# zsyOAOA/VIRNet

Measured on AMD Instinct MI355X. Metric: images/sec (256x256x3 denoise fwd), higher is better.
Workload: dtype f32 (3x3 conv products as split-fp16 MFMA pairs, f32 accumulate)

## Files before the change

### include/virnet_hip.h

```cpp
#ifndef VIRNET_HIP_H
#define VIRNET_HIP_H

#include <stddef.h>
#include <stdint.h>

#ifdef __cplusplus
extern "C" {
#endif

#define VIRNET_ABI_VERSION 5

int virnet_abi_version(void);
const char* virnet_last_error(void);
int virnet_device_count(void);

size_t virnet_packed_weight_floats(int ks, int cin_pad, int n_pad);
int virnet_pack_weight(const float* w, int kind, int cout, int cin, int ks, int cin_pad, int n_pad, int nrep,
                       float* packed, void* stream);

typedef struct virnet_conv_plan {
  int nrep;
  int n_pad;
  int cin_pad;
} virnet_conv_plan;
int virnet_conv_get_plan(int ks, int stride, int cin, int gemm_n, virnet_conv_plan* plan);

enum { VIRNET_EPI_NHWC = 0, VIRNET_EPI_CONVT = 1, VIRNET_EPI_NCHW = 2 };
enum { VIRNET_NCHW_PLAIN = 0, VIRNET_NCHW_ADD = 1, VIRNET_NCHW_EXPCLAMP = 2 };

typedef struct virnet_conv_desc {
  const float* x;
  const float* wpack;
  const float* bias;
  const float* res;
  const float* mul;
  const float* add;
  const float* mask;
  const float* in_mul;
  const float* in_add;
  float* y_raw;
  float* y_act;
  int n, h, w;
  int cin_pad;
  int cout;
  int n_pad;
  int nrep;
  int ks, stride;
  int epi;
  int nchw_op;
  int crop_h, crop_w;
  int res_sf;
  int in_act;
  float in_slope;
  float slope;
  float mask_slope;
  float clamp_lo, clamp_hi;
} virnet_conv_desc;

int virnet_conv_mfma(const virnet_conv_desc* d, void* stream);
int virnet_conv_mfma_variant(const virnet_conv_desc* d, int out[4]);

size_t virnet_wino_weight_floats(int cin_pad, int n_pad);
int virnet_pack_wino_weight(const float* w_oihw, int dgrad, int cout, int cin, int cin_pad, int n_pad, float* packed, void* stream);
int virnet_conv_wino(const virnet_conv_desc* d, void* stream);

size_t virnet_f16_weight_floats(int cin_pad, int n_pad);
int virnet_pack_f16_weight(const float* w_oihw, int dgrad, int cout, int cin, int cin_pad, int n_pad, float* packed, void* stream);
int virnet_conv_f16(const virnet_conv_desc* d, void* stream);
int virnet_pack_bf16_weight(const float* w_oihw, int dgrad, int cout, int cin, int cin_pad, int n_pad, float* packed, void* stream);
int virnet_conv_bf16(const virnet_conv_desc* d, void* stream);
size_t virnet_f16_convt_weight_floats(int cin, int cout);
int virnet_pack_f16_convt_weight(const float* w_iohw, int cout, int cin, float* packed, void* stream);

size_t virnet_wx4_weight_floats(int cin_pad, int n_pad);
int virnet_pack_wx4_weight(const float* w_oihw, int dgrad, int cout, int cin, int cin_pad, int n_pad, float* packed, void* stream);
int virnet_conv_wx4(const virnet_conv_desc* d, void* stream);
void virnet_conv_wx4_last_plan(int* out4);

enum { VIRNET_LAUNCH_WX4 = 0, VIRNET_LAUNCH_WX4H = 1, VIRNET_LAUNCH_WX4P = 2, VIRNET_LAUNCH_F16 = 3, VIRNET_LAUNCH_S2 = 4, VIRNET_LAUNCH_CONVT = 5 };
typedef struct virnet_conv_launch {
  int form, rows, ng, nrep, variant, slab_base, groups, persistent;
} virnet_conv_launch;
enum { VIRNET_PLAN_WX4 = 0, VIRNET_PLAN_F16 = 1, VIRNET_PLAN_BF16 = 2, VIRNET_PLAN_F16_ENTRY = 3 };
int virnet_conv_plan_query(int family, const virnet_conv_desc* d, int emit_rows, int n_cu,
                           virnet_conv_launch* out, int cap);

size_t virnet_exit_weight_floats(int cin_pad);
int virnet_pack_exit_weight(const float* w_oihw, int cout, int cin, int cin_pad, float* packed, void* stream);
int virnet_conv_exit(const virnet_conv_desc* d, void* stream);

int virnet_set_range_flag(int* device_flag);
int virnet_poison_on_flag(const int* device_flag, float* y, size_t n, void* stream);

typedef struct virnet_thin_desc {
  const float* x;
  const float* wpack;
  const float* bias;
  const float* res;
  float* y;
  int n, h, w, c, cout;
  int crop_h, crop_w;
  int op;
  int res_sf;
  float clamp_lo, clamp_hi;
} virnet_thin_desc;
size_t virnet_thin_weight_floats(int c_pad);
int virnet_pack_thin_weight(const float* w_oihw, int cout, int c, int c_pad, float* packed, void* stream);
int virnet_conv3x3_thin(const virnet_thin_desc* d, void* stream);

typedef struct virnet_pack_desc {
  const float* x;
  const float* vec;
  const float* map;
  float* out;
  int n, c0, h, w, sf;
  int ev;
  int em, mh, mw, msf, map_sqrt;
  int hp, wp;
  int zero_pad;
} virnet_pack_desc;
int virnet_pack_input(const virnet_pack_desc* d, void* stream);
int virnet_conv_f16_entry(const virnet_conv_desc* d, const virnet_pack_desc* e, void* stream);
size_t virnet_entry_weight_floats(int cin, int n_pad);
int virnet_pack_entry_weight(const float* w, int cout, int cin, int n_pad, float* packed, void* stream);
int virnet_conv_entry(const virnet_conv_desc* d, const virnet_pack_desc* e, void* stream);

typedef struct virnet_wgrad_desc {
  const float* x;
  const float* dy;
  const float* in_mul;
  const float* in_add;
  float* dw;
  int* counters;
  int n, h, w, cx, cy;
  int cin, cout;
  int ks, stride;
  int transposed;
  int in_act;
  float in_slope;
} virnet_wgrad_desc;
int virnet_conv_wgrad(const virnet_wgrad_desc* d, void* stream);
size_t virnet_chsplit_bytes(int n, int h, int w, int c);
size_t virnet_conv_wgrad_f16_scratch_bytes(int n, int h, int w, int cx, int cy);
size_t virnet_chsplit_colsum_bytes(int n, int h, int w, int c);
int virnet_chsplit(const float* x, int n, int h, int w, int c, int in_act, float in_slope, const float* in_mul, const float* in_add,
                   int bf16, void* out, float* col_scratch, float* db, int cvalid, void* stream);
int virnet_conv_wgrad_f16(const void* xt, const void* yt, float* dw, float* scratch, int n, int h, int w, int cx, int cy, int cin, int cout,
                          int bf16, void* stream);
int virnet_conv_wgrad_f16_db(const void* xt, const void* yt, float* dw, float* scratch, int n, int h, int w, int cx, int cy, int cin, int cout,
                             int bf16, const float* col, float* db, long nblk, int cvalid, void* stream);
size_t virnet_chsplit_s2_bytes(int n, int h, int w, int c);
size_t virnet_chsplit_s2_colsum_bytes(int n, int h, int w, int c);
int virnet_chsplit_s2(const float* x, int n, int h, int w, int c, int in_act, float in_slope, const float* in_mul, const float* in_add,
                      int bf16, void* out, float* col_scratch, float* db, int cvalid, void* stream);
size_t virnet_conv_wgrad_f16_s2_scratch_bytes(int n, int oh, int ow, int chi, int clo);
int virnet_conv_wgrad_f16_s2(const void* hi_t, const void* lo_t, float* dw, float* scratch, int n, int oh, int ow, int chi, int clo,
                             int cin, int cout, int mode, int bf16, void* stream);
typedef struct {
  int kg, nwv, pairs, split, run, nxs, nsteps;
} virnet_wgrad_f16_plan;
int virnet_conv_wgrad_f16_plan_query(int n, int h, int w, int cx, int cy, int mode, virnet_wgrad_f16_plan* out);
typedef struct virnet_t_emit {
  void* t_out;
  float* col;
  int act;
  float slope;
  int bf16;
  int rows;
} virnet_t_emit;
int virnet_conv_emit_ok(const virnet_conv_desc* d, int form, int* nblk);
int virnet_conv_f16_emit(const virnet_conv_desc* d, const virnet_t_emit* te, int bf16_operands, void* stream);
int virnet_conv_wx4_emit(const virnet_conv_desc* d, const virnet_t_emit* te, void* stream);
int virnet_colpart_reduce(const float* col, float* db, long nblk, int ncb, int cvalid, void* stream);
int virnet_sft_backward(const float* da, const float* x, const float* mul, const float* add, const float* res, float slope, float* dx,
                        float* dmul, float* dadd, int n, long hw, int c, void* stream);
int virnet_colsum(const float* dy, float* db, long npix, int c, int cvalid, void* stream);
int virnet_zero_stuff2(const float* dy, float* z, int n, int h, int w, int c, void* stream);
int virnet_space_to_depth2(const float* dy, float* out, int n, int h, int w, int c, void* stream);
int virnet_pack_input_backward(const float* drec, int crec, int chan, const float* map, float* dmap, int n, int h, int w, int hp,
                               int wp, int map_sqrt, int accumulate, void* stream);

typedef struct virnet_image_grad_desc {
  const float* dres;
  const float* ga;
  const float* wa;
  const float* gb;
  const float* wb;
  float* dx;
  int n, c0, h, w, sf;
  int hp, wp, ca, cina;
  int cb, cinb;
  int accumulate;
} virnet_image_grad_desc;
int virnet_image_grad(const virnet_image_grad_desc* d, void* stream);


int virnet_conv_head_s4(const float* x, const float* w, float* out, int n, int cin, int h, int w_, int cout, void* stream);
int virnet_conv_head_s4_wgrad(const float* x, const float* dy, float* dw, int n, int cin, int h, int w_, int cout, void* stream);
int virnet_conv_head_s4_dgrad(const float* dy, const float* w, float* dx, int n, int cin, int h, int w_, int cout, void* stream);

enum { VIRNET_GAP_MEAN = 0, VIRNET_GAP_EXPCLAMP = 1, VIRNET_GAP_KINFO = 2 };
int virnet_gap_nchw(const float* x, float* out, int n, int c, int h, int w, int finish, float lo, float hi, void* stream);

int virnet_ca_gate(const float* x, const float* w1, const float* b1, const float* w2, const float* b2, float* gate,
                   int n, int h, int w, int c, int cr, void* stream);

int virnet_scale_add(const float* hcv, const float* gate, const float* skip, float* out, int n, int hw, int c, void* stream);

int virnet_ca_scale_add(const float* hcv, const float* w1, const float* b1, const float* w2, const float* b2, const float* skip,
                        float* out, int n, int h, int w, int c, int cr, void* stream);

typedef struct virnet_knet_layer {
  const float *w1pack, *b1, *w2pack, *b2;
  const float *caw1, *cab1, *caw2, *cab2;
} virnet_knet_layer;
int virnet_knet_body(const float* x, float* y, const virnet_knet_layer* layers, int nlayers, int n, int h, int w, int c, int cr, void* stream);

typedef struct virnet_sft_weights {
  const float *w1, *b1;
  const float *w2, *b2;
  const float *wm, *bm;
  const float *wa, *ba;
  int e, nf1, nf2, nf;
} virnet_sft_weights;

int virnet_sft_vec(const float* vec, const virnet_sft_weights* wt, float* mul, float* add, int n, void* stream);
int virnet_sft_vec_multi(const float* vec, const virnet_sft_weights* wts, int nlayers, float* const* muls, float* const* adds, int n, void* stream);

int virnet_sft_apply(const float* raw, const float* rec, const virnet_sft_weights* wt, float* act, int n, int h, int w,
                     int step, int chan0, void* stream);

int virnet_quantize_u8(const float* x, uint8_t* out, size_t n, void* stream);
int virnet_rgb2y_u8(const uint8_t* rgb, uint8_t* y, int n, int h, int w, void* stream);
size_t virnet_psnr_ssim_workspace_bytes(int n, int c, int h, int w, int border, int ycbcr);
int virnet_psnr_ssim(const void* a, int a_f32, const void* b, int b_f32, int n, int c, int h, int w, int border, int ycbcr, int with_ssim,
                     const double* win11, void* workspace, int64_t* sse, int64_t* count, double* ssim, void* stream);

#define VIRNET_BORDER_REFLECT 0
#define VIRNET_BORDER_SYMMETRIC 1
int virnet_degrade_forward(const float* x, const float* kernel, float* y, int n, int c, int h, int w, int k, int sf, int border, int clip01,
                           void* stream);
int virnet_degrade_grad_image(const float* gy, const float* kernel, float* gx, int n, int c, int h, int w, int k, int sf, int border,
                              void* stream);
size_t virnet_degrade_grad_kernel_workspace_bytes(int n, int c, int h, int w, int k, int sf);
int virnet_degrade_grad_kernel(const float* gy, const float* x, float* gk, void* workspace, int n, int c, int h, int w, int k, int sf, int border,
                               void* stream);
int virnet_resample_axis(const void* in, int in_f64, void* out, int out_f64, const int32_t* idx, const double* wgt, int taps, long long outer,
                         int n_in, int n_out, long long inner, void* stream);

size_t virnet_elbo_workspace_bytes(int n, int c, int h, int w);
int virnet_elbo_value(const float* mu, const float* sigma_est, const float* im_noisy, const float* im_gt, const float* beta0,
                      const float* alpha0, const float* psi, float eps2, int with_klig, void* workspace, float* out4, int n, int c, int cs,
                      int cb, int h, int w, void* stream);
int virnet_elbo_grad(const float* mu, const float* sigma_est, const float* im_noisy, const float* im_gt, const float* beta0,
                     const float* alpha0, const float* grad_out, float eps2, double w_data, double w_klig, float* dmu, float* dsigma, int n,
                     int c, int cs, int cb, int h, int w, void* stream);
int virnet_noise_estimate(const float* im_noisy, const float* im_gt, const double* taps, float* out, int n, int c, int h, int w, int k,
                          float floor, void* stream);

size_t virnet_sisr_head_workspace_bytes(int n);
int virnet_sisr_head_forward(const float* kinfo_est, const float* kinfo_gt, const float* gamma, const float* rho_eps, const float* kappa0,
                             double r2, double penalty0, double penalty1, int k, int sf, int shift, void* workspace, float* kernel, float* out4,
                             int n, void* stream);
int virnet_sisr_head_backward(const float* kinfo_est, const float* kinfo_gt, const float* gamma, const float* rho_eps, const float* kappa0,
                              const float* grad_kernel, const float* grad_knet, double r2, double penalty0, double penalty1, int k, int sf,
                              int shift, float* dkinfo, int n, void* stream);
size_t virnet_sisr_hr_workspace_bytes(int n, int c, int h, int w);
int virnet_sisr_hr_value(const float* mu, const float* im_hr, const float* z_eps, double eps2, void* workspace, float* zz, float* out1, int n,
                         int c, int h, int w, void* stream);
int virnet_sisr_hr_grad(const float* mu, const float* im_hr, const float* grad_zz, const float* grad_rnet, double eps2, float* dmu, int n, int c,
                        int h, int w, void* stream);
size_t virnet_sisr_lr_workspace_bytes(int n, int c, int h, int w);
int virnet_sisr_lr_value(const float* y, const float* im_lr, const float* sigma_est, const float* sigma_prior, const float* alpha0,
                         const float* psi, void* workspace, double* stats, float* out2, int n, int c, int h, int w, int cs, int fs, int cp, int fp,
                         void* stream);
int virnet_sisr_lr_grad(const float* y, const float* im_lr, const float* sigma_est, const float* sigma_prior, const float* alpha0,
                        const double* stats, const float* grad_lh, const float* grad_snet, float* dy, float* dsigma, int n, int c, int h, int w,
                        int cs, int fs, int cp, int fp, void* stream);
int virnet_sisr_finish(const float* lh, const float* kl_rnet, const float* kl_snet, const float* kl_knet, float* loss, void* stream);

#ifdef __cplusplus
}
#endif
#endif
```

### virnet_amd/_native.py

```python
from __future__ import annotations

import ctypes as C
import os
import threading

import torch

_HERE = os.path.dirname(os.path.abspath(__file__))
LIB_PATH = os.environ.get("VIRNET_HIP_LIB") or os.path.join(_HERE, "lib", "libvirnet_hip.so")
ABI_VERSION = 5

c_float_p = C.POINTER(C.c_float)


class ConvPlan(C.Structure):
    _fields_ = [("nrep", C.c_int), ("n_pad", C.c_int), ("cin_pad", C.c_int)]


class ConvDesc(C.Structure):
    _fields_ = [
        ("x", C.c_void_p), ("wpack", C.c_void_p), ("bias", C.c_void_p), ("res", C.c_void_p),
        ("mul", C.c_void_p), ("add", C.c_void_p), ("mask", C.c_void_p), ("in_mul", C.c_void_p), ("in_add", C.c_void_p),
        ("y_raw", C.c_void_p), ("y_act", C.c_void_p),
        ("n", C.c_int), ("h", C.c_int), ("w", C.c_int), ("cin_pad", C.c_int), ("cout", C.c_int),
        ("n_pad", C.c_int), ("nrep", C.c_int), ("ks", C.c_int), ("stride", C.c_int), ("epi", C.c_int),
        ("nchw_op", C.c_int), ("crop_h", C.c_int), ("crop_w", C.c_int), ("res_sf", C.c_int),
        ("in_act", C.c_int), ("in_slope", C.c_float), ("slope", C.c_float), ("mask_slope", C.c_float), ("clamp_lo", C.c_float), ("clamp_hi", C.c_float),
    ]


class ConvLaunch(C.Structure):
    _fields_ = [(k, C.c_int) for k in ("form", "rows", "ng", "nrep", "variant", "slab_base", "groups", "persistent")]


class WgradF16Plan(C.Structure):
    _fields_ = [(k, C.c_int) for k in ("kg", "nwv", "pairs", "split", "run", "nxs", "nsteps")]


class TEmit(C.Structure):
    _fields_ = [("t_out", C.c_void_p), ("col", C.c_void_p), ("act", C.c_int), ("slope", C.c_float), ("bf16", C.c_int), ("rows", C.c_int)]


class PackDesc(C.Structure):
    _fields_ = [
        ("x", C.c_void_p), ("vec", C.c_void_p), ("map", C.c_void_p), ("out", C.c_void_p),
        ("n", C.c_int), ("c0", C.c_int), ("h", C.c_int), ("w", C.c_int), ("sf", C.c_int),
        ("ev", C.c_int),
        ("em", C.c_int), ("mh", C.c_int), ("mw", C.c_int), ("msf", C.c_int), ("map_sqrt", C.c_int),
        ("hp", C.c_int), ("wp", C.c_int), ("zero_pad", C.c_int),
    ]


class ImageGradDesc(C.Structure):
    _fields_ = [
        ("dres", C.c_void_p), ("ga", C.c_void_p), ("wa", C.c_void_p), ("gb", C.c_void_p), ("wb", C.c_void_p), ("dx", C.c_void_p),
        ("n", C.c_int), ("c0", C.c_int), ("h", C.c_int), ("w", C.c_int), ("sf", C.c_int),
        ("hp", C.c_int), ("wp", C.c_int), ("ca", C.c_int), ("cina", C.c_int),
        ("cb", C.c_int), ("cinb", C.c_int), ("accumulate", C.c_int),
    ]


class ThinDesc(C.Structure):
    _fields_ = [
        ("x", C.c_void_p), ("wpack", C.c_void_p), ("bias", C.c_void_p), ("res", C.c_void_p), ("y", C.c_void_p),
        ("n", C.c_int), ("h", C.c_int), ("w", C.c_int), ("c", C.c_int), ("cout", C.c_int),
        ("crop_h", C.c_int), ("crop_w", C.c_int), ("op", C.c_int), ("res_sf", C.c_int),
        ("clamp_lo", C.c_float), ("clamp_hi", C.c_float),
    ]


class WgradDesc(C.Structure):
    _fields_ = [
        ("x", C.c_void_p), ("dy", C.c_void_p), ("in_mul", C.c_void_p), ("in_add", C.c_void_p), ("dw", C.c_void_p),
        ("counters", C.c_void_p), ("n", C.c_int), ("h", C.c_int), ("w", C.c_int), ("cx", C.c_int), ("cy", C.c_int),
        ("cin", C.c_int), ("cout", C.c_int), ("ks", C.c_int), ("stride", C.c_int), ("transposed", C.c_int),
        ("in_act", C.c_int), ("in_slope", C.c_float),
    ]


class KnetLayer(C.Structure):
    _fields_ = [(k, C.c_void_p) for k in ("w1pack", "b1", "w2pack", "b2", "caw1", "cab1", "caw2", "cab2")]


class SftWeights(C.Structure):
    _fields_ = [
        ("w1", C.c_void_p), ("b1", C.c_void_p), ("w2", C.c_void_p), ("b2", C.c_void_p),
        ("wm", C.c_void_p), ("bm", C.c_void_p), ("wa", C.c_void_p), ("ba", C.c_void_p),
        ("e", C.c_int), ("nf1", C.c_int), ("nf2", C.c_int), ("nf", C.c_int),
    ]


EPI_NHWC, EPI_CONVT, EPI_NCHW = 0, 1, 2
GAP_MEAN, GAP_EXPCLAMP, GAP_KINFO = 0, 1, 2
NCHW_PLAIN, NCHW_ADD, NCHW_EXPCLAMP = 0, 1, 2
PLAN_WX4, PLAN_F16, PLAN_BF16, PLAN_F16_ENTRY = 0, 1, 2, 3

SYMBOLS = [
    ("virnet_abi_version", C.c_int, []),
    ("virnet_last_error", C.c_char_p, []),
    ("virnet_device_count", C.c_int, []),
    ("virnet_packed_weight_floats", C.c_size_t, [C.c_int, C.c_int, C.c_int]),
    ("virnet_pack_weight", C.c_int, [C.c_void_p, C.c_int, C.c_int, C.c_int, C.c_int, C.c_int, C.c_int, C.c_int,
                                     C.c_void_p, C.c_void_p]),
    ("virnet_conv_get_plan", C.c_int, [C.c_int, C.c_int, C.c_int, C.c_int, C.POINTER(ConvPlan)]),
    ("virnet_conv_mfma", C.c_int, [C.POINTER(ConvDesc), C.c_void_p]),
    ("virnet_conv_mfma_variant", C.c_int, [C.POINTER(ConvDesc), C.POINTER(C.c_int * 4)]),
    ("virnet_wino_weight_floats", C.c_size_t, [C.c_int, C.c_int]),
    ("virnet_pack_wino_weight", C.c_int, [C.c_void_p, C.c_int, C.c_int, C.c_int, C.c_int, C.c_int, C.c_void_p, C.c_void_p]),
    ("virnet_conv_wino", C.c_int, [C.POINTER(ConvDesc), C.c_void_p]),
    ("virnet_f16_weight_floats", C.c_size_t, [C.c_int, C.c_int]),
    ("virnet_pack_f16_weight", C.c_int, [C.c_void_p, C.c_int, C.c_int, C.c_int, C.c_int, C.c_int, C.c_void_p, C.c_void_p]),
    ("virnet_conv_f16", C.c_int, [C.POINTER(ConvDesc), C.c_void_p]),
    ("virnet_wx4_weight_floats", C.c_size_t, [C.c_int, C.c_int]),
    ("virnet_pack_wx4_weight", C.c_int, [C.c_void_p, C.c_int, C.c_int, C.c_int, C.c_int, C.c_int, C.c_void_p, C.c_void_p]),
    ("virnet_conv_wx4", C.c_int, [C.POINTER(ConvDesc), C.c_void_p]),
    ("virnet_conv_wx4_last_plan", None, [C.POINTER(C.c_int)]),
    ("virnet_conv_plan_query", C.c_int, [C.c_int, C.POINTER(ConvDesc), C.c_int, C.c_int, C.POINTER(ConvLaunch), C.c_int]),
    ("virnet_exit_weight_floats", C.c_size_t, [C.c_int]),
    ("virnet_pack_exit_weight", C.c_int, [C.c_void_p, C.c_int, C.c_int, C.c_int, C.c_void_p, C.c_void_p]),
    ("virnet_conv_exit", C.c_int, [C.POINTER(ConvDesc), C.c_void_p]),
    ("virnet_set_range_flag", C.c_int, [C.c_void_p]),
    ("virnet_poison_on_flag", C.c_int, [C.c_void_p, C.c_void_p, C.c_size_t, C.c_void_p]),
    ("virnet_pack_bf16_weight", C.c_int, [C.c_void_p, C.c_int, C.c_int, C.c_int, C.c_int, C.c_int, C.c_void_p, C.c_void_p]),
    ("virnet_conv_bf16", C.c_int, [C.POINTER(ConvDesc), C.c_void_p]),
    ("virnet_f16_convt_weight_floats", C.c_size_t, [C.c_int, C.c_int]),
    ("virnet_pack_f16_convt_weight", C.c_int, [C.c_void_p, C.c_int, C.c_int, C.c_void_p, C.c_void_p]),
    ("virnet_pack_input", C.c_int, [C.POINTER(PackDesc), C.c_void_p]),
    ("virnet_conv_f16_entry", C.c_int, [C.POINTER(ConvDesc), C.POINTER(PackDesc), C.c_void_p]),
    ("virnet_entry_weight_floats", C.c_size_t, [C.c_int, C.c_int]),
    ("virnet_pack_entry_weight", C.c_int, [C.c_void_p, C.c_int, C.c_int, C.c_int, C.c_void_p, C.c_void_p]),
    ("virnet_conv_entry", C.c_int, [C.POINTER(ConvDesc), C.POINTER(PackDesc), C.c_void_p]),
    ("virnet_thin_weight_floats", C.c_size_t, [C.c_int]),
    ("virnet_pack_thin_weight", C.c_int, [C.c_void_p, C.c_int, C.c_int, C.c_int, C.c_void_p, C.c_void_p]),
    ("virnet_conv3x3_thin", C.c_int, [C.POINTER(ThinDesc), C.c_void_p]),
    ("virnet_conv_wgrad", C.c_int, [C.POINTER(WgradDesc), C.c_void_p]),
    ("virnet_sft_backward", C.c_int, [C.c_void_p, C.c_void_p, C.c_void_p, C.c_void_p, C.c_void_p, C.c_float, C.c_void_p, C.c_void_p, C.c_void_p,
                                      C.c_int, C.c_long, C.c_int, C.c_void_p]),
    ("virnet_chsplit_bytes", C.c_size_t, [C.c_int, C.c_int, C.c_int, C.c_int]),
    ("virnet_conv_wgrad_f16_scratch_bytes", C.c_size_t, [C.c_int, C.c_int, C.c_int, C.c_int, C.c_int]),
    ("virnet_chsplit_colsum_bytes", C.c_size_t, [C.c_int, C.c_int, C.c_int, C.c_int]),
    ("virnet_chsplit", C.c_int, [C.c_void_p, C.c_int, C.c_int, C.c_int, C.c_int, C.c_int, C.c_float, C.c_void_p, C.c_void_p, C.c_int,
                                 C.c_void_p, C.c_void_p, C.c_void_p, C.c_int, C.c_void_p]),
    ("virnet_conv_wgrad_f16", C.c_int, [C.c_void_p, C.c_void_p, C.c_void_p, C.c_void_p, C.c_int, C.c_int, C.c_int, C.c_int, C.c_int, C.c_int, C.c_int,
                                        C.c_int, C.c_void_p]),
    ("virnet_chsplit_s2_bytes", C.c_size_t, [C.c_int, C.c_int, C.c_int, C.c_int]),
    ("virnet_chsplit_s2_colsum_bytes", C.c_size_t, [C.c_int, C.c_int, C.c_int, C.c_int]),
    ("virnet_chsplit_s2", C.c_int, [C.c_void_p, C.c_int, C.c_int, C.c_int, C.c_int, C.c_int, C.c_float, C.c_void_p, C.c_void_p, C.c_int,
                                    C.c_void_p, C.c_void_p, C.c_void_p, C.c_int, C.c_void_p]),
    ("virnet_conv_wgrad_f16_s2_scratch_bytes", C.c_size_t, [C.c_int, C.c_int, C.c_int, C.c_int, C.c_int]),
    ("virnet_conv_wgrad_f16_s2", C.c_int, [C.c_void_p, C.c_void_p, C.c_void_p, C.c_void_p, C.c_int, C.c_int, C.c_int, C.c_int, C.c_int, C.c_int,
                                           C.c_int, C.c_int, C.c_int, C.c_void_p]),
    ("virnet_conv_wgrad_f16_plan_query", C.c_int, [C.c_int, C.c_int, C.c_int, C.c_int, C.c_int, C.c_int, C.POINTER(WgradF16Plan)]),
    ("virnet_conv_emit_ok", C.c_int, [C.POINTER(ConvDesc), C.c_int, C.POINTER(C.c_int)]),
    ("virnet_conv_f16_emit", C.c_int, [C.POINTER(ConvDesc), C.POINTER(TEmit), C.c_int, C.c_void_p]),
    ("virnet_conv_wx4_emit", C.c_int, [C.POINTER(ConvDesc), C.POINTER(TEmit), C.c_void_p]),
    ("virnet_colpart_reduce", C.c_int, [C.c_void_p, C.c_void_p, C.c_long, C.c_int, C.c_int, C.c_void_p]),
    ("virnet_conv_wgrad_f16_db", C.c_int, [C.c_void_p, C.c_void_p, C.c_void_p, C.c_void_p, C.c_int, C.c_int, C.c_int, C.c_int, C.c_int, C.c_int, C.c_int,
                                           C.c_int, C.c_void_p, C.c_void_p, C.c_long, C.c_int, C.c_void_p]),
    ("virnet_colsum", C.c_int, [C.c_void_p, C.c_void_p, C.c_long, C.c_int, C.c_int, C.c_void_p]),
    ("virnet_zero_stuff2", C.c_int, [C.c_void_p, C.c_void_p, C.c_int, C.c_int, C.c_int, C.c_int, C.c_void_p]),
    ("virnet_space_to_depth2", C.c_int, [C.c_void_p, C.c_void_p, C.c_int, C.c_int, C.c_int, C.c_int, C.c_void_p]),
    ("virnet_pack_input_backward", C.c_int, [C.c_void_p, C.c_int, C.c_int, C.c_void_p, C.c_void_p, C.c_int, C.c_int, C.c_int, C.c_int,
                                             C.c_int, C.c_int, C.c_int, C.c_void_p]),
    ("virnet_image_grad", C.c_int, [C.POINTER(ImageGradDesc), C.c_void_p]),
    ("virnet_conv_head_s4", C.c_int, [C.c_void_p, C.c_void_p, C.c_void_p, C.c_int, C.c_int, C.c_int, C.c_int, C.c_int,
                                      C.c_void_p]),
    ("virnet_conv_head_s4_wgrad", C.c_int, [C.c_void_p, C.c_void_p, C.c_void_p, C.c_int, C.c_int, C.c_int, C.c_int, C.c_int,
                                            C.c_void_p]),
    ("virnet_conv_head_s4_dgrad", C.c_int, [C.c_void_p, C.c_void_p, C.c_void_p, C.c_int, C.c_int, C.c_int, C.c_int, C.c_int,
                                            C.c_void_p]),
    ("virnet_gap_nchw", C.c_int, [C.c_void_p, C.c_void_p, C.c_int, C.c_int, C.c_int, C.c_int, C.c_int, C.c_float,
                                  C.c_float, C.c_void_p]),
    ("virnet_ca_gate", C.c_int, [C.c_void_p, C.c_void_p, C.c_void_p, C.c_void_p, C.c_void_p, C.c_void_p, C.c_int, C.c_int,
                                 C.c_int, C.c_int, C.c_int, C.c_void_p]),
    ("virnet_knet_body", C.c_int, [C.c_void_p, C.c_void_p, C.c_void_p, C.c_int, C.c_int, C.c_int, C.c_int, C.c_int, C.c_int, C.c_void_p]),
    ("virnet_scale_add", C.c_int, [C.c_void_p, C.c_void_p, C.c_void_p, C.c_void_p, C.c_int, C.c_int, C.c_int, C.c_void_p]),
    ("virnet_ca_scale_add", C.c_int, [C.c_void_p] * 7 + [C.c_int] * 5 + [C.c_void_p]),
    ("virnet_sft_vec", C.c_int, [C.c_void_p, C.POINTER(SftWeights), C.c_void_p, C.c_void_p, C.c_int, C.c_void_p]),
    ("virnet_sft_vec_multi", C.c_int, [C.c_void_p, C.POINTER(SftWeights), C.c_int, C.POINTER(C.c_void_p), C.POINTER(C.c_void_p), C.c_int, C.c_void_p]),
    ("virnet_sft_apply", C.c_int, [C.c_void_p, C.c_void_p, C.POINTER(SftWeights), C.c_void_p, C.c_int, C.c_int, C.c_int,
                                   C.c_int, C.c_int, C.c_void_p]),
    ("virnet_quantize_u8", C.c_int, [C.c_void_p, C.c_void_p, C.c_size_t, C.c_void_p]),
    ("virnet_rgb2y_u8", C.c_int, [C.c_void_p, C.c_void_p, C.c_int, C.c_int, C.c_int, C.c_void_p]),
    ("virnet_psnr_ssim_workspace_bytes", C.c_size_t, [C.c_int] * 6),
    ("virnet_psnr_ssim", C.c_int, [C.c_void_p, C.c_int, C.c_void_p, C.c_int] + [C.c_int] * 7 + [C.POINTER(C.c_double)] + [C.c_void_p] * 5),
    ("virnet_degrade_forward", C.c_int, [C.c_void_p] * 3 + [C.c_int] * 8 + [C.c_void_p]),
    ("virnet_degrade_grad_image", C.c_int, [C.c_void_p] * 3 + [C.c_int] * 7 + [C.c_void_p]),
    ("virnet_degrade_grad_kernel_workspace_bytes", C.c_size_t, [C.c_int] * 6),
    ("virnet_degrade_grad_kernel", C.c_int, [C.c_void_p] * 4 + [C.c_int] * 7 + [C.c_void_p]),
    ("virnet_resample_axis", C.c_int, [C.c_void_p, C.c_int, C.c_void_p, C.c_int, C.c_void_p, C.c_void_p, C.c_int, C.c_longlong, C.c_int, C.c_int,
                                       C.c_longlong, C.c_void_p]),
    ("virnet_elbo_workspace_bytes", C.c_size_t, [C.c_int] * 4),
    ("virnet_elbo_value", C.c_int, [C.c_void_p] * 7 + [C.c_float, C.c_int, C.c_void_p, C.c_void_p] + [C.c_int] * 6 + [C.c_void_p]),
    ("virnet_elbo_grad", C.c_int, [C.c_void_p] * 7 + [C.c_float, C.c_double, C.c_double, C.c_void_p, C.c_void_p] + [C.c_int] * 6 + [C.c_void_p]),
    ("virnet_noise_estimate", C.c_int, [C.c_void_p] * 4 + [C.c_int] * 5 + [C.c_float, C.c_void_p]),
    ("virnet_sisr_head_workspace_bytes", C.c_size_t, [C.c_int]),
    ("virnet_sisr_head_forward", C.c_int, [C.c_void_p] * 5 + [C.c_double] * 3 + [C.c_int] * 3 + [C.c_void_p] * 3 + [C.c_int, C.c_void_p]),
    ("virnet_sisr_head_backward", C.c_int, [C.c_void_p] * 7 + [C.c_double] * 3 + [C.c_int] * 3 + [C.c_void_p, C.c_int, C.c_void_p]),
    ("virnet_sisr_hr_workspace_bytes", C.c_size_t, [C.c_int] * 4),
    ("virnet_sisr_hr_value", C.c_int, [C.c_void_p] * 3 + [C.c_double] + [C.c_void_p] * 3 + [C.c_int] * 4 + [C.c_void_p]),
    ("virnet_sisr_hr_grad", C.c_int, [C.c_void_p] * 4 + [C.c_double, C.c_void_p] + [C.c_int] * 4 + [C.c_void_p]),
    ("virnet_sisr_lr_workspace_bytes", C.c_size_t, [C.c_int] * 4),
    ("virnet_sisr_lr_value", C.c_int, [C.c_void_p] * 9 + [C.c_int] * 8 + [C.c_void_p]),
    ("virnet_sisr_lr_grad", C.c_int, [C.c_void_p] * 10 + [C.c_int] * 8 + [C.c_void_p]),
    ("virnet_sisr_finish", C.c_int, [C.c_void_p] * 6),
]

_lib = None


class NativeLibraryError(RuntimeError):
    pass


def load() -> C.CDLL:
    global _lib
    if _lib is not None:
        return _lib
    if not os.path.exists(LIB_PATH):
        raise NativeLibraryError(
            f"{LIB_PATH} not found: the VIRNet HIP kernels are not built. Run `python -c 'import __graft_entry__ as g; "
            f"g.build()'` (or `make -C virnet_amd/csrc`) -- there is no CPU fallback for the product path.")
    lib = C.CDLL(LIB_PATH)
    for name, restype, argtypes in SYMBOLS:
        try:
            fn = getattr(lib, name)
        except AttributeError as e:
            raise NativeLibraryError(f"{LIB_PATH} does not export {name}; rebuild it") from e
        fn.restype = restype
        fn.argtypes = argtypes
    if lib.virnet_abi_version() != ABI_VERSION:
        raise NativeLibraryError(f"{LIB_PATH}: ABI {lib.virnet_abi_version()} != expected {ABI_VERSION}; rebuild it")
    _lib = lib
    return lib


def check(rc: int, what: str = "") -> None:
    if rc != 0:
        msg = load().virnet_last_error()
        raise RuntimeError(f"libvirnet_hip {what}: {msg.decode() if msg else 'unknown error'}")


def ptr(t) -> int:
    return 0 if t is None else t.data_ptr()


tls = threading.local()
capture_lock = threading.RLock()


def stream_handle() -> int:
    cached = getattr(tls, "stream_cache", None)
    if cached is not None:
        return cached
    return torch.cuda.current_stream().cuda_stream
```

### virnet_amd/csrc/conv_exit.hip

```cpp
#include "conv_f16_common.h"

namespace {
using namespace virnet;

constexpr int EX_TH = 8, EX_TW = 32;
constexpr int EX_HW = EX_TW + 2;
constexpr int EX_HPX = (EX_TH + 2) * EX_HW;
constexpr int EX_BLK = (EX_HPX + 31) / 32;
constexpr int EX_ZS = EX_BLK * 32 + 4;

template <int NCH>
__global__ __launch_bounds__(256) void conv_exit_kernel(const FArgs a) {
  extern __shared__ __attribute__((aligned(16))) char smem[];
  const int nch = NCH ? NCH : (a.Cin >> 4);
  char* const a_lds = smem;
  float* const z_lds = reinterpret_cast<float*>(smem + nch * 2048);

  const int xcd = blockIdx.x & 7, q = blockIdx.x >> 3;
  const int tile = xcd * a.tiles_per_xcd + q;
  if (q >= a.tiles_per_xcd || tile >= a.ntiles) return;
  const int img = fast_div(tile, a.mg_tpi);
  const int trem = tile - img * (a.ntx * a.nty);
  const int ty = fast_div(trem, a.mg_ntx), tx = trem - ty * a.ntx;
  const int oy0 = ty * EX_TH, ox0 = tx * EX_TW;

  const int tid = threadIdx.x, lane = tid & 63, wave = __builtin_amdgcn_readfirstlane(tid >> 6);
  const int l31 = lane & 31, lhi = lane >> 5;
  const int nrows = a.cout * 9;
  TSTAMP(0);

  if constexpr (NCH != 0) {
    f32x4 wv[NCH / 2];
#pragma unroll
    for (int i = 0; i < NCH / 2; ++i) wv[i] = *reinterpret_cast<const f32x4*>(a.wimg + i * 4096 + tid * 16);
#pragma unroll
    for (int i = 0; i < NCH / 2; ++i) *reinterpret_cast<f32x4*>(a_lds + i * 4096 + tid * 16) = wv[i];
  } else {
    for (int i = tid * 16; i < nch * 2048; i += 256 * 16) *reinterpret_cast<f32x4*>(a_lds + i) = *reinterpret_cast<const f32x4*>(a.wimg + i);
  }
  __syncthreads();
  TSTAMP(1);

  const int oyl = tid >> 5, oxl = tid & 31;
  const int oy = oy0 + oyl, ox = ox0 + oxl;
  const bool inside = oy < a.crop_h && ox < a.crop_w;
  const size_t plane = (size_t)a.crop_h * a.crop_w;
  const size_t o0 = (size_t)img * a.cout * plane + (size_t)oy * a.crop_w + ox;
  float scv[27], bsv[3];
#pragma unroll
  for (int i = 0; i < 27; ++i) scv[i] = a.inv_scale[i];
#pragma unroll
  for (int c = 0; c < 3; ++c) bsv[c] = (a.bias && c < a.cout) ? a.bias[c] : 0.f;
  float rv[3] = {0.f, 0.f, 0.f};
  if (a.nchw_op == VIRNET_NCHW_ADD && inside) {
    const int rw = a.crop_w / a.res_sf;
    const size_t rplane = (size_t)(a.crop_h / a.res_sf) * rw;
    const size_t r0 = (size_t)img * a.cout * rplane + (size_t)(oy / a.res_sf) * rw + ox / a.res_sf;
#pragma unroll
    for (int c = 0; c < 3; ++c)
      if (c < a.cout) rv[c] = a.res[a.res_sf > 1 ? r0 + c * rplane : o0 + c * plane];
  }

  const float* const ximg = a.x + (size_t)img * a.H * a.W * a.Cin;
  float amax = 0.f;
  auto pixel_of = [&](int blk) -> const float* {
    const int p = blk * 32 + l31;
    const int hy = p / EX_HW, hx = p - hy * EX_HW;
    const int gy = oy0 - 1 + hy, gx = ox0 - 1 + hx;
    const bool valid = blk < EX_BLK && p < EX_HPX && (unsigned)gy < (unsigned)a.H && (unsigned)gx < (unsigned)a.W;
    return valid ? ximg + ((size_t)gy * a.W + gx) * a.Cin + lhi * 8 : nullptr;
  };
  auto mma = [&](f32x16& acc, int c, f32x4 v0, f32x4 v1) {
    if (a.in_act) { v0 = lrelu4(v0, a.in_slope); v1 = lrelu4(v1, a.in_slope); }
    range_note(amax, v0, v1);
    h8 bh, bl;
    split8(v0, v1, bh, bl);
    const h8 ah = *reinterpret_cast<const h8*>(a_lds + c * 2048 + lane * 16);
    const h8 al = *reinterpret_cast<const h8*>(a_lds + c * 2048 + 1024 + lane * 16);
    acc = __builtin_amdgcn_mfma_f32_32x32x16_f16(al, bh, acc, 0, 0, 0);
    acc = __builtin_amdgcn_mfma_f32_32x32x16_f16(ah, bl, acc, 0, 0, 0);
    acc = __builtin_amdgcn_mfma_f32_32x32x16_f16(ah, bh, acc, 0, 0, 0);
  };
  auto put_z = [&](int blk, const f32x16& acc) {
    const int p = blk * 32 + l31;
#pragma unroll
    for (int r = 0; r < 16; ++r) {
      const int row = 8 * (r >> 2) + 4 * lhi + (r & 3);
      z_lds[min(row, nrows) * EX_ZS + p] = acc[r];
    }
  };
  if constexpr (NCH != 0) {
    const auto xrs = __builtin_amdgcn_make_buffer_rsrc(const_cast<float*>(ximg), 0, a.H * a.W * a.Cin * 4, 0x00020000);
    auto pixel_off = [&](int blk) -> unsigned {
      const int p = blk * 32 + l31;
      const int hy = p / EX_HW, hx = p - hy * EX_HW;
      const int gy = oy0 - 1 + hy, gx = ox0 - 1 + hx;
      const bool valid = p < EX_HPX && (unsigned)gy < (unsigned)a.H && (unsigned)gx < (unsigned)a.W;
      return valid ? (unsigned)(((gy * a.W + gx) * a.Cin + lhi * 8) * 4) : 0x80000000u;
    };
    auto request = [&](unsigned off, f32x4 (&v0)[NCH], f32x4 (&v1)[NCH]) {
#pragma unroll
      for (int c = 0; c < NCH; ++c) {
        v0[c] = __builtin_bit_cast(f32x4, __builtin_amdgcn_raw_buffer_load_b128(xrs, off + c * 64, 0, 0));
        v1[c] = __builtin_bit_cast(f32x4, __builtin_amdgcn_raw_buffer_load_b128(xrs, off + c * 64 + 16, 0, 0));
      }
    };
    auto compute = [&](int blk, f32x4 (&v0)[NCH], f32x4 (&v1)[NCH]) {
      f32x16 acc;
#pragma unroll
      for (int r = 0; r < 16; ++r) acc[r] = 0.f;
#pragma unroll
      for (int c = 0; c < NCH; ++c) mma(acc, c, v0[c], v1[c]);
      put_z(blk, acc);
    };
    static_assert(EX_BLK > 8 && EX_BLK <= 12, "three blocks per wave at most, two at least");
    f32x4 p0[NCH], p1[NCH], q0[NCH], q1[NCH];
    const bool third = wave + 8 < EX_BLK;
    request(pixel_off(wave), p0, p1);
    request(pixel_off(wave + 4), q0, q1);
    compute(wave, p0, p1);
    if (third) request(pixel_off(wave + 8), p0, p1);
    compute(wave + 4, q0, q1);
    if (third) compute(wave + 8, p0, p1);
  } else {
    for (int blk = wave; blk < EX_BLK; blk += 4) {
      const float* const px = pixel_of(blk);
      f32x16 acc;
#pragma unroll
      for (int r = 0; r < 16; ++r) acc[r] = 0.f;
      for (int c = 0; c < nch; ++c) {
        f32x4 v0 = f32x4{0.f, 0.f, 0.f, 0.f}, v1 = v0;
        if (px) {
          v0 = *reinterpret_cast<const f32x4*>(px + c * 16);
          v1 = *reinterpret_cast<const f32x4*>(px + c * 16 + 4);
        }
        mma(acc, c, v0, v1);
      }
      put_z(blk, acc);
    }
  }
  TSTAMP(2);
  range_report(a.range_flag, amax);
  __syncthreads();
  TSTAMP(3);
#ifdef VIRNET_F16_TIMING
  if (a.tlog && tid == 0) {
    a.tlog[(size_t)blockIdx.x * 8 + 5] = __builtin_amdgcn_s_getreg((31 << 11) | (0 << 6) | 4);
    a.tlog[(size_t)blockIdx.x * 8 + 6] = __builtin_amdgcn_s_getreg((31 << 11) | (0 << 6) | 20);
  }
#endif

  if (!inside) return;
  float outv[3];
#pragma unroll
  for (int c = 0; c < 3; ++c) {
    float v = bsv[c];
    const float* const zc = z_lds + (c < a.cout ? c * 9 : 0) * EX_ZS + oyl * EX_HW + oxl;
#pragma unroll
    for (int dy = 0; dy < 3; ++dy)
#pragma unroll
      for (int dx = 0; dx < 3; ++dx) v += zc[(dy * 3 + dx) * EX_ZS + dy * EX_HW + dx] * scv[c * 9 + dy * 3 + dx];
    if (a.nchw_op == VIRNET_NCHW_ADD) v += rv[c];
    else if (a.nchw_op == VIRNET_NCHW_EXPCLAMP) v = expf(fminf(fmaxf(v, a.clamp_lo), a.clamp_hi));
    outv[c] = v;
  }
#pragma unroll
  for (int c = 0; c < 3; ++c)
    if (c < a.cout) a.y_raw[o0 + c * plane] = outv[c];
#ifdef VIRNET_F16_TIMING
  asm volatile("s_waitcnt vmcnt(0)" ::: "memory");
#endif
  TSTAMP(4);
}

__global__ void pack_exit_kernel(const float* __restrict__ w, int cout, int cin, int cin_pad, float* __restrict__ inv_scale, char* __restrict__ img) {
  const int nrows = cout * 9;
  __shared__ int eb[32];
  if (threadIdx.x < 32) {
    const int row = threadIdx.x;
    float m = 0.f;
    if (row < nrows) {
      const int c = row / 9, t = row - c * 9;
      for (int k = 0; k < cin; ++k) m = fmaxf(m, fabsf(w[((size_t)c * cin + k) * 9 + t]));
    }
    int e = 0;
    if (m > 0.f) { frexpf(m, &e); e = 14 - e; }
    e = max(-100, min(100, e));
    eb[row] = e;
    inv_scale[row] = ldexpf(1.f, -e);
  }
  __syncthreads();
  for (int i = threadIdx.x; i < 32 * cin_pad; i += blockDim.x) {
    const int row = i / cin_pad, k = i - row * cin_pad;
    float v = 0.f;
    if (row < nrows && k < cin) {
      const int c = row / 9, t = row - c * 9;
      v = ldexpf(w[((size_t)c * cin + k) * 9 + t], eb[row]);
    }
    const int chunk = k >> 4, kk = k & 15;
    const size_t base = (size_t)chunk * 2048 + (size_t)(row + 32 * (kk >> 3)) * 16 + (kk & 7) * 2;
    const _Float16 hi = (_Float16)v;
    *reinterpret_cast<_Float16*>(img + base) = hi;
    *reinterpret_cast<_Float16*>(img + base + 1024) = (_Float16)(v - (float)hi);
  }
}

template <int NCH>
int launch_exit(FArgs k, hipStream_t st) {
  const int nch = k.Cin >> 4;
  const int lds = nch * 2048 + (k.cout * 9 + 1) * EX_ZS * 4;
  static unsigned long long attr_done = 0;
  auto kern = conv_exit_kernel<NCH>;
  if (virnet::first_use_on_device(attr_done)) {
    hipError_t e = hipFuncSetAttribute(reinterpret_cast<const void*>(kern), hipFuncAttributeMaxDynamicSharedMemorySize, 160 * 1024);
    if (e != hipSuccess) return virnet::set_error("hipFuncSetAttribute(conv_exit): %s", hipGetErrorString(e));
  }
  hipLaunchKernelGGL(kern, dim3((unsigned)(8 * k.tiles_per_xcd)), dim3(256), lds, st, k);
  return virnet::check_launch("conv_exit launch");
}

#ifdef VIRNET_F16_TIMING
long long* g_xlog = nullptr;
#endif
}

#ifdef VIRNET_F16_TIMING
extern "C" void virnet_debug_exit_timing_buffer(void* p) { g_xlog = static_cast<long long*>(p); }
#endif

extern "C" size_t virnet_exit_weight_floats(int cin_pad) { return 32 + (size_t)cin_pad * 32; }

extern "C" int virnet_pack_exit_weight(const float* w, int cout, int cin, int cin_pad, float* packed, void* stream) {
  VIRNET_REQUIRE(w && packed, "virnet_pack_exit_weight: NULL pointer");
  VIRNET_REQUIRE(cout >= 1 && cout * 9 <= 32, "virnet_pack_exit_weight: cout=%d: the (channel, tap) rows must fit one 32-row block (cout <= 3)", cout);
  VIRNET_REQUIRE(cin >= 1 && cin_pad % 16 == 0 && cin_pad >= cin, "virnet_pack_exit_weight: cin_pad=%d does not cover cin=%d", cin_pad, cin);
  hipLaunchKernelGGL(pack_exit_kernel, dim3(1), dim3(256), 0, static_cast<hipStream_t>(stream), w, cout, cin, cin_pad, packed,
                     reinterpret_cast<char*>(packed + 32));
  return virnet::check_launch("pack_exit launch");
}

extern "C" int virnet_conv_exit(const virnet_conv_desc* d, void* stream) {
  VIRNET_REQUIRE(d != nullptr, "virnet_conv_exit: desc is NULL");
  VIRNET_REQUIRE(d->x && d->wpack && d->y_raw, "virnet_conv_exit: x / wpack / y_raw is NULL");
  VIRNET_REQUIRE(d->ks == 3 && d->stride == 1 && d->epi == VIRNET_EPI_NCHW, "virnet_conv_exit: only the stride-1 3x3 conv with planar store (ks=%d stride=%d epi=%d)",
                 d->ks, d->stride, d->epi);
  VIRNET_REQUIRE(d->n > 0 && d->h > 0 && d->w > 0, "virnet_conv_exit: empty input n=%d h=%d w=%d", d->n, d->h, d->w);
  VIRNET_REQUIRE(d->cout >= 1 && d->cout * 9 <= 32, "virnet_conv_exit: cout=%d (the (channel, tap) rows must fit one 32-row block: cout <= 3)", d->cout);
  VIRNET_REQUIRE(d->cin_pad >= 16 && d->cin_pad % 16 == 0 && d->cin_pad <= 1024, "virnet_conv_exit: cin_pad=%d", d->cin_pad);
  VIRNET_REQUIRE(d->crop_h >= 1 && d->crop_h <= d->h && d->crop_w >= 1 && d->crop_w <= d->w, "virnet_conv_exit: crop %d x %d outside %d x %d", d->crop_h, d->crop_w, d->h, d->w);
  VIRNET_REQUIRE(d->nchw_op != VIRNET_NCHW_ADD || d->res, "virnet_conv_exit: VIRNET_NCHW_ADD without res");
  VIRNET_REQUIRE(d->res_sf >= 1 && d->crop_h % d->res_sf == 0 && d->crop_w % d->res_sf == 0, "virnet_conv_exit: res_sf=%d does not divide the crop", d->res_sf);
  VIRNET_REQUIRE(!d->mask && !d->mul && !d->in_mul && !d->y_act, "virnet_conv_exit: plain planar epilogue only");
  VIRNET_REQUIRE((long)d->h * d->w * d->cin_pad * 4 < (1L << 31), "virnet_conv_exit: one image's input (%d x %d x %d fp32) must stay below 2 GB (32-bit buffer offsets)", d->h, d->w, d->cin_pad);
  FArgs k{};
  k.x = d->x; k.inv_scale = d->wpack; k.wimg = reinterpret_cast<const char*>(d->wpack + 32);
  k.bias = d->bias; k.res = d->res; k.y_raw = d->y_raw;
  k.N = d->n; k.H = d->h; k.W = d->w; k.Cin = d->cin_pad; k.cout = d->cout;
  k.in_act = d->in_act; k.in_slope = d->in_slope;
  k.nchw_op = d->nchw_op; k.crop_h = d->crop_h; k.crop_w = d->crop_w; k.res_sf = d->res_sf; k.clamp_lo = d->clamp_lo; k.clamp_hi = d->clamp_hi;
  k.range_flag = virnet::range_flag_ptr();
#ifdef VIRNET_F16_TIMING
  k.tlog = g_xlog;
#endif
  k.nty = (d->crop_h + EX_TH - 1) / EX_TH;
  k.ntx = (d->crop_w + EX_TW - 1) / EX_TW;
  k.ntiles = k.N * k.nty * k.ntx;
  k.tiles_per_xcd = (k.ntiles + 7) / 8;
  VIRNET_REQUIRE((unsigned long long)k.ntiles * (unsigned)(k.ntx * k.nty) < (1ull << 32), "virnet_conv_exit: %d tiles exceed the index arithmetic of one launch", k.ntiles);
  k.mg_ntx = div_magic(k.ntx);
  k.mg_tpi = div_magic(k.ntx * k.nty);
  hipStream_t st = static_cast<hipStream_t>(stream);
  const int nch = d->cin_pad >> 4;
  if (nch == 6) return launch_exit<6>(k, st);
  if (nch == 4) return launch_exit<4>(k, st);
  VIRNET_REQUIRE(nch * 2048 + 33 * EX_ZS * 4 <= 160 * 1024, "virnet_conv_exit: cin_pad=%d does not fit LDS", d->cin_pad);
  return launch_exit<0>(k, st);
}
```

### virnet_amd/csrc/pack.hip

```cpp
#include "common.h"
#include "../../include/virnet_hip.h"

namespace {

__global__ void pack_weight_kernel(const float* __restrict__ w, float* __restrict__ out, int kind, int cout, int cin, int ks,
                                   int cin_pad, int n_pad, int nrep, size_t total) {
  const int ntaps = ks * ks;
  const int nchunks = cin_pad / 16;
  for (size_t i = (size_t)blockIdx.x * blockDim.x + threadIdx.x; i < total; i += (size_t)gridDim.x * blockDim.x) {
    size_t r = i;
    const int rr = (int)(r & 3); r >>= 2;
    const int lane = (int)(r & 63); r >>= 6;
    const int nr = (int)(r % nrep); r /= nrep;
    const int j = (int)(r & 1); r >>= 1;
    const int t = (int)(r % ntaps); r /= ntaps;
    const int c = (int)(r % nchunks); r /= nchunks;
    const int cb = (int)r;
    const int ci = c * 16 + 8 * j + 4 * (lane >> 5) + rr;
    const int n = (cb * nrep + nr) * 32 + (lane & 31);
    float v = 0.f;
    if (kind == 0) {
      if (ci < cin && n < cout) v = w[((size_t)n * cin + ci) * ntaps + t];
    } else if (kind == 1) {
      const int ab = n / cout, co = n - ab * cout;
      if (ci < cin && ab < 4) v = w[((size_t)ci * cout + co) * 4 + ab];
    } else if (kind == 2) {
      if (ci < cout && n < cin) v = w[((size_t)ci * cin + n) * ntaps + (ntaps - 1 - t)];
    } else {
      const int ab = ci / cout, co = ci - ab * cout;
      if (n < cin && ab < 4) v = w[((size_t)n * cout + co) * 4 + ab];
    }
    out[i] = v;
  }
}

__device__ __forceinline__ int reflect(int i, int n) { return i < n ? i : 2 * n - 2 - i; }

__global__ void pack_input_kernel(const virnet_pack_desc d) {
  const size_t npix = (size_t)d.n * d.hp * d.wp;
  const int HU = d.h * d.sf, WU = d.w * d.sf;
  for (size_t i = (size_t)blockIdx.x * blockDim.x + threadIdx.x; i < npix * 4; i += (size_t)gridDim.x * blockDim.x) {
    const int q = (int)(i & 3);
    const size_t pix = i >> 2;
    const int x = (int)(pix % d.wp);
    const int y = (int)((pix / d.wp) % d.hp);
    const int n = (int)(pix / ((size_t)d.wp * d.hp));
    const int ry = reflect(y, HU), rx = reflect(x, WU);
    const bool dead = d.zero_pad && (y >= HU || x >= WU);
    float v[4];
#pragma unroll
    for (int k = 0; k < 4; ++k) {
      int c = q * 4 + k;
      float val = 0.f;
      if (c < d.c0) {
        val = d.x[(((size_t)n * d.c0 + c) * d.h + ry / d.sf) * d.w + rx / d.sf];
      } else if ((c -= d.c0) < d.ev) {
        val = d.vec[(size_t)n * d.ev + c];
      } else if ((c -= d.ev) < d.em) {
        val = d.map[(((size_t)n * d.em + c) * d.mh + ry / d.msf) * d.mw + rx / d.msf];
        if (d.map_sqrt) val = sqrtf(val);
      }
      v[k] = dead ? 0.f : val;
    }
    reinterpret_cast<float4*>(d.out)[i] = make_float4(v[0], v[1], v[2], v[3]);
  }
}

__global__ void zero_stuff2_kernel(const float4* __restrict__ dy, float4* __restrict__ z, int h, int w, int c4, size_t total) {
  for (size_t i = (size_t)blockIdx.x * blockDim.x + threadIdx.x; i < total; i += (size_t)gridDim.x * blockDim.x) {
    const int q = (int)(i % c4);
    size_t p = i / c4;
    const int x = (int)(p % (2 * w)); p /= 2 * w;
    const int y = (int)(p % (2 * h));
    const size_t n = p / (2 * h);
    float4 v = make_float4(0.f, 0.f, 0.f, 0.f);
    if (!((x | y) & 1)) v = dy[((n * h + (y >> 1)) * w + (x >> 1)) * c4 + q];
    z[i] = v;
  }
}

__global__ void space_to_depth2_kernel(const float4* __restrict__ dy, float4* __restrict__ out, int h, int w, int c4, size_t total) {
  for (size_t i = (size_t)blockIdx.x * blockDim.x + threadIdx.x; i < total; i += (size_t)gridDim.x * blockDim.x) {
    const int q = (int)(i % c4);
    size_t p = i / c4;
    const int ab = (int)(p & 3); p >>= 2;
    const int x = (int)(p % w); p /= w;
    const int y = (int)(p % h);
    const size_t n = p / h;
    out[i] = dy[((n * 2 * h + 2 * y + (ab >> 1)) * 2 * w + 2 * x + (ab & 1)) * c4 + q];
  }
}

__global__ void pack_input_backward_kernel(const float* __restrict__ drec, int crec, int chan, const float* __restrict__ map,
                                           float* __restrict__ dmap, int h, int w, int hp, int wp, int map_sqrt, int accumulate,
                                           size_t total) {
  for (size_t i = (size_t)blockIdx.x * blockDim.x + threadIdx.x; i < total; i += (size_t)gridDim.x * blockDim.x) {
    const int x = (int)(i % w), y = (int)((i / w) % h);
    const size_t n = i / ((size_t)w * h);
    const int ym = 2 * h - 2 - y, xm = 2 * w - 2 - x;
    const bool my = ym >= h && ym < hp, mx = xm >= w && xm < wp;
    const float* base = drec + (n * hp * (size_t)wp) * crec + chan;
    float g = base[((size_t)y * wp + x) * crec];
    if (my) g += base[((size_t)ym * wp + x) * crec];
    if (mx) g += base[((size_t)y * wp + xm) * crec];
    if (my && mx) g += base[((size_t)ym * wp + xm) * crec];
    if (map_sqrt) g *= 0.5f / sqrtf(map[i]);
    dmap[i] = accumulate ? dmap[i] + g : g;
  }
}

}

static int grid_for(size_t total) { return (int)((total + 255) / 256 > 8192 ? 8192 : (total + 255) / 256); }

extern "C" int virnet_zero_stuff2(const float* dy, float* z, int n, int h, int w, int c, void* stream) {
  VIRNET_REQUIRE(dy && z && n > 0 && h > 0 && w > 0 && c > 0 && c % 4 == 0, "virnet_zero_stuff2: bad arguments");
  const size_t total = (size_t)n * 2 * h * 2 * w * (c / 4);
  hipLaunchKernelGGL(zero_stuff2_kernel, dim3(grid_for(total)), dim3(256), 0, static_cast<hipStream_t>(stream),
                     reinterpret_cast<const float4*>(dy), reinterpret_cast<float4*>(z), h, w, c / 4, total);
  return virnet::check_launch("zero_stuff2 launch");
}

extern "C" int virnet_space_to_depth2(const float* dy, float* out, int n, int h, int w, int c, void* stream) {
  VIRNET_REQUIRE(dy && out && n > 0 && h > 0 && w > 0 && c > 0 && c % 4 == 0, "virnet_space_to_depth2: bad arguments");
  const size_t total = (size_t)n * h * w * 4 * (c / 4);
  hipLaunchKernelGGL(space_to_depth2_kernel, dim3(grid_for(total)), dim3(256), 0, static_cast<hipStream_t>(stream),
                     reinterpret_cast<const float4*>(dy), reinterpret_cast<float4*>(out), h, w, c / 4, total);
  return virnet::check_launch("space_to_depth2 launch");
}

extern "C" int virnet_pack_input_backward(const float* drec, int crec, int chan, const float* map, float* dmap, int n, int h, int w,
                                          int hp, int wp, int map_sqrt, int accumulate, void* stream) {
  VIRNET_REQUIRE(drec && dmap && n > 0 && h > 0 && w > 0 && hp >= h && wp >= w && hp - h < h && wp - w < w,
                 "virnet_pack_input_backward: bad shape %dx%d -> %dx%d", h, w, hp, wp);
  VIRNET_REQUIRE(chan >= 0 && chan < crec, "virnet_pack_input_backward: channel %d of %d", chan, crec);
  VIRNET_REQUIRE(!map_sqrt || map, "virnet_pack_input_backward: map_sqrt without map");
  const size_t total = (size_t)n * h * w;
  hipLaunchKernelGGL(pack_input_backward_kernel, dim3(grid_for(total)), dim3(256), 0, static_cast<hipStream_t>(stream), drec, crec,
                     chan, map, dmap, h, w, hp, wp, map_sqrt, accumulate, total);
  return virnet::check_launch("pack_input_backward launch");
}

extern "C" size_t virnet_packed_weight_floats(int ks, int cin_pad, int n_pad) {
  return (size_t)ks * ks * cin_pad * n_pad;
}

extern "C" int virnet_pack_weight(const float* w, int kind, int cout, int cin, int ks, int cin_pad, int n_pad, int nrep,
                                  float* packed, void* stream) {
  VIRNET_REQUIRE(w && packed, "virnet_pack_weight: NULL pointer");
  VIRNET_REQUIRE(kind >= 0 && kind <= 3, "virnet_pack_weight: kind=%d", kind);
  VIRNET_REQUIRE(nrep >= 1 && n_pad % (32 * nrep) == 0 && cin_pad % 16 == 0, "virnet_pack_weight: n_pad=%d nrep=%d cin_pad=%d", n_pad, nrep, cin_pad);
  const int rows = kind == 0 ? cout : kind == 1 ? 4 * cout : cin;
  const int contr = kind <= 1 ? cin : kind == 2 ? cout : 4 * cout;
  VIRNET_REQUIRE(n_pad >= rows && cin_pad >= contr, "virnet_pack_weight: n_pad=%d / cin_pad=%d do not cover %d rows x %d channels (kind %d)",
                 n_pad, cin_pad, rows, contr, kind);
  VIRNET_REQUIRE((kind == 1 || kind == 3) ? ks == 2 : (ks == 3 || ks == 1), "virnet_pack_weight: ks=%d for kind %d", ks, kind);
  const int gemm_ks = (kind == 1 || kind == 3) ? 1 : ks;
  const size_t total = virnet_packed_weight_floats(gemm_ks, cin_pad, n_pad);
  const int grid = (int)((total + 255) / 256 > 4096 ? 4096 : (total + 255) / 256);
  hipLaunchKernelGGL(pack_weight_kernel, dim3(grid), dim3(256), 0, static_cast<hipStream_t>(stream), w, packed, kind, cout, cin,
                     gemm_ks, cin_pad, n_pad, nrep, total);
  return virnet::check_launch("pack_weight launch");
}

extern "C" int virnet_pack_input(const virnet_pack_desc* d, void* stream) {
  VIRNET_REQUIRE(d && d->x && d->out, "virnet_pack_input: NULL pointer");
  VIRNET_REQUIRE(d->n > 0 && d->h > 0 && d->w > 0 && d->sf >= 1, "virnet_pack_input: bad shape n=%d h=%d w=%d sf=%d", d->n, d->h,
                 d->w, d->sf);
  VIRNET_REQUIRE(d->c0 >= 1 && d->ev >= 0 && d->em >= 0 && d->c0 + d->ev + d->em <= 16,
                 "virnet_pack_input: %d+%d+%d channels do not fit a 16-channel record", d->c0, d->ev, d->em);
  VIRNET_REQUIRE(d->ev == 0 || d->vec, "virnet_pack_input: ev=%d without vec", d->ev);
  VIRNET_REQUIRE(d->em == 0 || (d->map && d->msf >= 1), "virnet_pack_input: em=%d without map/msf", d->em);
  const int HU = d->h * d->sf, WU = d->w * d->sf;
  VIRNET_REQUIRE(d->hp >= HU && d->wp >= WU && d->hp - HU < HU && d->wp - WU < WU,
                 "virnet_pack_input: reflect pad %dx%d -> %dx%d needs pad < dim", HU, WU, d->hp, d->wp);
  VIRNET_REQUIRE(d->em == 0 || (d->mh * d->msf == HU && d->mw * d->msf == WU),
                 "virnet_pack_input: map %dx%d x%d does not match image %dx%d", d->mh, d->mw, d->msf, HU, WU);
  const size_t total = (size_t)d->n * d->hp * d->wp * 4;
  const int grid = (int)((total + 255) / 256 > 8192 ? 8192 : (total + 255) / 256);
  hipLaunchKernelGGL(pack_input_kernel, dim3(grid), dim3(256), 0, static_cast<hipStream_t>(stream), *d);
  return virnet::check_launch("pack_input launch");
}
```

### virnet_amd/engine.py

```python
from __future__ import annotations

from typing import List, Optional, Tuple

import torch

from . import _native as nat
from . import ops

Tensor = torch.Tensor

LOG_MAX = 4.605170185988092
LOG_MIN = -23.025850929940457
K_LOG_MIN = -9.210340371976182


def _prep(x: Tensor, chn: int, name: str = "x") -> Tensor:
    if x.dim() != 4:
        raise ValueError(f"{name} must be [N,C,H,W], got {tuple(x.shape)}")
    if x.shape[1] != chn:
        raise ValueError(f"{name} has {x.shape[1]} channels, the network was built for {chn}")
    if not x.is_cuda:
        raise RuntimeError(f"{name} is on {x.device}: the VIRNet HIP path runs on a ROCm device only (no CPU fallback)")
    if x.dtype != torch.float32:
        raise TypeError(f"{name} must be float32 (the reference is fp32 end to end), got {x.dtype}")
    return x.detach().contiguous()


def _ceil_to(v: int, m: int) -> int:
    return (v + m - 1) // m * m


def snet_forward(snet, x: Tensor, mode: str = "raw") -> Tensor:
    x = _prep(x, snet.in_channels)
    n, _, h, w = x.shape
    cur = ops.conv_entry(x, snet.conv1.packed(), h, w, want_act=True, slope=0.25)
    for key in sorted(snet.mid_layer.keys(), key=int):
        _, cur = ops.conv_mfma(cur, snet.mid_layer[key].packed(), want_raw=False, want_act=True, slope=0.25)
    last = snet.conv_last
    if snet.noise_avg:
        raw = ops.conv_planar(cur, last, (h, w))
        fin = ops.GAP_EXPCLAMP if mode == "sigma" else ops.GAP_MEAN
        return ops.gap_nchw(raw, fin, (LOG_MIN, LOG_MAX)).view(n, -1, 1, 1)
    if mode == "sigma":
        return ops.conv_planar(cur, last, (h, w), op=nat.NCHW_EXPCLAMP, clamp=(LOG_MIN, LOG_MAX))
    return ops.conv_planar(cur, last, (h, w))


def knet_forward(knet, x: Tensor) -> Tensor:
    x = _prep(x, knet.in_nc)
    n, _, h, w = x.shape
    cur = ops.conv_head_s4(x, knet.head.weight)
    persistent = (ops._f16_family() and cur.shape[3] == 64 and max(cur.shape[1:3]) <= ops.KNET_BODY_MAX and len(knet.body) > 0
                  and ops._env("VIRNET_KNET_PERSISTENT", "1") != "0")
    if persistent:
        cur = ops.knet_body(cur, [(rb.body["0"].packed(), rb.body["2"].packed(), rb.body["3"].body["0"].weight, rb.body["3"].body["0"].bias,
                                   rb.body["3"].body["2"].weight, rb.body["3"].body["2"].bias) for rb in knet.body])
    for rb in (() if persistent else knet.body):
        _, a = ops.conv_mfma(cur, rb.body["0"].packed(), want_raw=False, want_act=True, slope=0.2)
        hcv, _ = ops.conv_mfma(a, rb.body["2"].packed(), want_raw=True)
        ca = rb.body["3"].body
        cur = ops.ca_scale_add(hcv, ca["0"].weight, ca["0"].bias, ca["2"].weight, ca["2"].bias, cur)
    oh, ow = cur.shape[1:3]
    raw = ops.conv_planar(cur, knet.tail["0"], (oh, ow))
    return ops.gap_nchw(raw, ops.GAP_KINFO, (K_LOG_MIN, LOG_MAX)).view(n, -1, 1, 1)


class _Cond:

    def __init__(self, vec: Optional[Tensor], rec: Optional[Tensor], chan0: int, nchan: int):
        self.vec, self.rec, self.chan0, self.nchan = vec, rec, chan0, nchan
        self.pre = {}

    def sft(self, att):
        got = self.pre.get(id(att))
        return got if got is not None else ops.sft_vec(self.vec, att)


def _res_block(x_raw: Tensor, blk, cond: Optional[_Cond], level: int) -> Tensor:
    sft = cond is not None and blk.extra_chn > 0
    c1, c2 = blk.conv1.packed(), blk.conv2.packed()
    if not sft:
        _, f1a = ops.conv_mfma(x_raw, c1, in_slope=0.2, want_raw=False, want_act=True, slope=0.2)
    elif cond.vec is not None:
        mul1, add1 = cond.sft(blk.sft1)
        mul2, add2 = cond.sft(blk.sft2)
        _, f1a = ops.conv_mfma(x_raw, c1, in_slope=0.2, in_mul=mul1, in_add=add1, mul=mul2, add=add2, want_raw=False,
                               want_act=True, slope=0.2)
    else:
        a1 = ops.sft_apply(x_raw, cond.rec, cond.chan0, cond.nchan, 1 << level, blk.sft1)
        f1, _ = ops.conv_mfma(a1, c1, want_raw=True)
        f1a = ops.sft_apply(f1, cond.rec, cond.chan0, cond.nchan, 1 << level, blk.sft2)
    out, _ = ops.conv_mfma(f1a, c2, res=x_raw, want_raw=True)
    return out


def rnet_forward(rnet, x_in: Tensor, *, extra_map: Optional[Tensor] = None, extra_vec: Optional[Tensor] = None,
                 sf: int = 1, map_sf: int = 1, map_sqrt: bool = False) -> Tensor:
    x_in = _prep(x_in, rnet.in_chn)
    mode = rnet.extra_mode
    n, _, h0, w0 = x_in.shape
    H, W = h0 * sf, w0 * sf
    m = 1 << (rnet.depth - 1)
    Hp, Wp = _ceil_to(H, m), _ceil_to(W, m)
    ev = 0 if extra_vec is None else extra_vec.shape[1]
    em = 0 if extra_map is None else extra_map.shape[1]
    if mode != "null":
        if ev + em != rnet.extra_chn:
            raise ValueError(f"conditioning has {ev + em} channels, the network was built for {rnet.extra_chn}")
        if extra_map is not None:
            extra_map = _prep(extra_map, em, "extra maps")
        if extra_vec is not None:
            extra_vec = extra_vec.detach().contiguous()
    feed_head = mode in ("input", "both")
    feed_down = mode in ("down", "both")
    cond = None
    rec = None
    if feed_down:
        if extra_map is None:
            cond = _Cond(extra_vec, None, 0, ev)
        else:
            rec = ops.pack_input(x_in, Hp, Wp, sf=sf, vec=extra_vec if feed_head else None,
                                 map_=extra_map if feed_head else None, map_sf=map_sf, map_sqrt=map_sqrt)
            crec = rec if feed_head else ops.pack_input(x_in, Hp, Wp, sf=sf, vec=extra_vec, map_=extra_map,
                                                        map_sf=map_sf, map_sqrt=map_sqrt)
            cond = _Cond(None, crec, rnet.in_chn, ev + em)
    if rec is not None:
        x, _ = ops.conv_mfma(rec, rnet.head.packed(), want_raw=True)
    else:
        x = ops.conv_entry(x_in, rnet.head.packed(), Hp, Wp, sf=sf, vec=extra_vec if feed_head else None,
                           map_=extra_map if feed_head else None, map_sf=map_sf, map_sqrt=map_sqrt)
    if cond is not None and cond.vec is not None and ops._env("VIRNET_SFT_MULTI", "1") != "0":
        atts = [a for lvl in rnet.down_path for blk in lvl.body if blk.extra_chn > 0 for a in (blk.sft1, blk.sft2)]
        if atts:
            cond.pre = {id(a): ma for a, ma in zip(atts, ops.sft_vec_multi(cond.vec, atts))}
    bridges: List[Tensor] = []
    for ii, lvl in enumerate(rnet.down_path):
        for blk in lvl.body:
            x = _res_block(x, blk, cond, ii)
        if ii + 1 < len(rnet.down_path):
            bridges.append(x)
            x, _ = ops.conv_mfma(x, lvl.downsampler.packed(), stride=2, want_raw=True)
    for jj, up in enumerate(rnet.up_path):
        x, _ = ops.conv_mfma(x, up.upsampler.packed(), res=bridges[-jj - 1], want_raw=True)
        for blk in up.body:
            x = _res_block(x, blk, None, 0)
    return ops.conv_planar(x, rnet.tail, (H, W), op=nat.NCHW_ADD, res=x_in, res_sf=sf)


FP32_FORM = "wino"


class RangeOverflowRepaired(RuntimeWarning):
    """A forward of the deferred guard mode left fp16's range: its outputs were NaN on the device until the repair that this warning
    announces (the same input repeated with the fp32 kernels, written into the same output tensors)."""


_GUARD_WARNING = ("VIRNet HIP path: an activation left fp16's range in a split-fp16 convolution (|x| >= 65504, or >= ~6.5e3 in the "
                  "Winograd form); the forward was repeated with the fp32 kernels")
MAX_PENDING = 2


def guard_check_mode() -> str:
    mode = ops._env("VIRNET_GUARD_CHECK", "sync")
    if mode not in ("sync", "deferred"):
        raise ValueError(f"VIRNET_GUARD_CHECK={mode!r}: expected sync or deferred")
    return mode


def _pending_list() -> list:
    lst = getattr(nat.tls, "guard_pending", None)
    if lst is None:
        lst = nat.tls.guard_pending = []
    return lst


def _settle(block: bool, keep: int = 0) -> None:
    import warnings
    pend = _pending_list()
    while pend:
        pinned, ev, run, outs, dev, stream = pend[0]
        if not ev.query():
            if not block or len(pend) <= keep:
                return
            ev.synchronize()
        pend.pop(0)
        overflowed = bool(int(pinned[0]))
        _pinned_pool().append(pinned)
        if overflowed:
            _GUARD_STATS["reruns"] += 1
            with torch.no_grad(), torch.cuda.device(dev), torch.cuda.stream(stream), ops.forward_scope(form=FP32_FORM):
                res = run()
                for o, r in zip(outs, res if isinstance(res, tuple) else (res,)):
                    o.copy_(r)
            warnings.warn(_GUARD_WARNING + " (deferred check: its outputs were NaN until now)", RangeOverflowRepaired, stacklevel=4)


def _pinned_pool() -> list:
    pool = getattr(nat.tls, "guard_pinned", None)
    if pool is None:
        pool = nat.tls.guard_pinned = []
    return pool


def guard_poll(block: bool = True) -> None:
    _settle(block)


def _range_guarded(run, x: Tensor):
    import warnings
    guarded = ops._f16_family() and ops.range_guard_enabled() and not torch.cuda.is_current_stream_capturing()
    deferred = guarded and guard_check_mode() == "deferred"
    if guarded:
        _settle(block=False)
        flag = ops.range_flag(x.device)
        flag.zero_()
    with ops.forward_scope():
        out = run()
    if deferred:
        outs = out if isinstance(out, tuple) else (out,)
        for o in outs:
            ops.poison_on_flag(flag, o)
        pool = _pinned_pool()
        if pool:
            pinned = pool.pop()
        else:
            with nat.capture_lock:
                pinned = torch.zeros(1, dtype=torch.int32).pin_memory()
        pinned.copy_(flag, non_blocking=True)
        ev = torch.cuda.Event()
        ev.record()
        _pending_list().append((pinned, ev, run, outs, x.device, torch.cuda.current_stream()))
        _settle(block=True, keep=MAX_PENDING)
    elif guarded and ops.range_overflowed(x.device):
        warnings.warn(_GUARD_WARNING, RuntimeWarning, stacklevel=3)
        _GUARD_STATS["reruns"] += 1
        with ops.forward_scope(form=FP32_FORM):
            out = run()
    if guarded:
        _GUARD_STATS["forwards"] += 1
    return out


_GUARD_STATS = {"forwards": 0, "reruns": 0}


def guard_stats(reset: bool = False) -> dict:
    out = dict(_GUARD_STATS)
    if reset:
        _GUARD_STATS["forwards"] = _GUARD_STATS["reruns"] = 0
    return out


def denoise_forward(net, x: Tensor) -> Tuple[Tensor, Tensor]:
    x = _prep(x, net.SNet.in_channels)
    with torch.cuda.device(x.device):
        return _range_guarded(lambda: _denoise_forward(net, x), x)


def _denoise_forward(net, x: Tensor) -> Tuple[Tensor, Tensor]:
    sigma = snet_forward(net.SNet, x, mode="sigma")
    if net.noise_cond:
        if net.SNet.noise_avg:
            raise RuntimeError("VIRAttResUNet(noise_avg=True, noise_cond=True): the [N,C,1,1] variance cannot be "
                               "padded or concatenated with the image (same failure as the reference)")
        mu = rnet_forward(net.RNet, x, extra_map=sigma, map_sqrt=True)
    else:
        mu = rnet_forward(net.RNet, x)
    return mu, sigma


def sisr_forward(net, x: Tensor, sf) -> Tuple[Tensor, Tensor, Tensor]:
    x = _prep(x, net.SNet.in_channels)
    with torch.cuda.device(x.device):
        return _range_guarded(lambda: _sisr_forward(net, x, sf), x)


def _sisr_forward(net, x: Tensor, sf) -> Tuple[Tensor, Tensor, Tensor]:
    if int(sf) != sf or sf < 1:
        raise ValueError(f"sf must be a positive integer, got {sf}")
    sf = int(sf)
    n = x.shape[0]
    sigma = snet_forward(net.SNet, x, mode="sigma")
    kinfo = knet_forward(net.KNet, x)
    vec_parts, emap = [], None
    if net.kernel_cond:
        vec_parts.append(kinfo.view(n, -1))
    if net.noise_cond:
        if net.noise_avg:
            vec_parts.append(sigma.view(n, -1).sqrt())
        else:
            emap = sigma
    vec = torch.cat(vec_parts, 1).contiguous() if vec_parts else None
    mu = rnet_forward(net.RNet, x, extra_map=emap, extra_vec=vec, sf=sf, map_sf=sf, map_sqrt=True)
    return mu, kinfo.view(n, -1), sigma
```

### virnet_amd/networks/AttResUNet.py

```python
from __future__ import annotations

from typing import Optional, Sequence

import torch
from torch import nn

from .params import ConvParam
from .. import engine


class AttLayer(nn.Module):

    def __init__(self, out_chn: int = 64, extra_chn: int = 4):
        super().__init__()
        nf1, nf2 = out_chn // 8, out_chn // 4
        self.out_chn, self.extra_chn = out_chn, extra_chn
        self.conv1 = ConvParam(extra_chn, nf1, 1)
        self.conv2 = ConvParam(nf1, nf2, 1)
        self.mul_conv = ConvParam(nf2, out_chn, 1)
        self.add_conv = ConvParam(nf2, out_chn, 1)


class AttResBlock(nn.Module):

    def __init__(self, nf: int = 64, extra_chn: int = 4):
        super().__init__()
        self.nf, self.extra_chn = nf, extra_chn
        if extra_chn > 0:
            self.sft1 = AttLayer(nf, extra_chn)
            self.sft2 = AttLayer(nf, extra_chn)
        self.conv1 = ConvParam(nf, nf, 3)
        self.conv2 = ConvParam(nf, nf, 3)


class DownBlock(nn.Module):

    def __init__(self, in_chn: int = 64, out_chn: int = 128, extra_chn: int = 4, n_resblocks: int = 1,
                 downsample: bool = True):
        super().__init__()
        self.body = nn.ModuleList([AttResBlock(in_chn, extra_chn) for _ in range(n_resblocks)])
        self.downsampler = ConvParam(in_chn, out_chn, 3, stride=2) if downsample else nn.Identity()


class UpBlock(nn.Module):

    def __init__(self, in_chn: int = 128, out_chn: int = 64, n_resblocks: int = 1):
        super().__init__()
        self.upsampler = ConvParam(in_chn, out_chn, 2, transposed=True, stride=2)
        self.body = nn.ModuleList([AttResBlock(nf=out_chn, extra_chn=0) for _ in range(n_resblocks)])


class AttResUNet(nn.Module):
    def __init__(self, in_chn: int = 3, extra_chn: int = 4, out_chn: int = 3, n_resblocks: int = 2,
                 n_feat: Sequence[int] = (64, 128, 196, 256), extra_mode: str = "Input"):
        super().__init__()
        assert isinstance(n_feat, (tuple, list))
        self.depth = len(n_feat)
        self.extra_mode = extra_mode.lower()
        assert self.extra_mode in ["null", "input", "down", "both"]
        self.in_chn, self.extra_chn, self.out_chn = in_chn, extra_chn, out_chn
        self.n_feat, self.n_resblocks = list(n_feat), n_resblocks
        for c in n_feat:
            if c % 32:
                raise ValueError(f"n_feat={list(n_feat)}: the MFMA kernels tile output channels in blocks of 32 "
                                 f"(all reference configurations use multiples of 32)")
        head_in = in_chn if self.extra_mode in ("down", "null") else in_chn + extra_chn
        if head_in > 16:
            raise ValueError("image + conditioning channels must fit one 16-channel pixel record")
        self.head = ConvParam(head_in, n_feat[0], 3)
        extra_down = extra_chn if self.extra_mode in ("down", "both") else 0
        self.down_path = nn.ModuleList()
        for ii in range(self.depth):
            last = ii + 1 == self.depth
            self.down_path.append(DownBlock(n_feat[ii], n_feat[ii] if last else n_feat[ii + 1], extra_chn=extra_down,
                                            n_resblocks=n_resblocks, downsample=not last))
        self.up_path = nn.ModuleList()
        for jj in reversed(range(self.depth - 1)):
            self.up_path.append(UpBlock(n_feat[jj + 1], n_feat[jj], n_resblocks))
        self.tail = ConvParam(n_feat[0], out_chn, 3)

    def forward(self, x_in: torch.Tensor, extra_maps_in: Optional[torch.Tensor]) -> torch.Tensor:
        return engine.rnet_forward(self, x_in, extra_map=extra_maps_in)
```

### virnet_amd/ops.py

```python
from __future__ import annotations

import ctypes as C
import os
from dataclasses import dataclass
from typing import Optional, Tuple

import torch

from . import _native as nat

Tensor = torch.Tensor


@dataclass
class PackedWeight:
    w: Tensor
    bias: Optional[Tensor]
    ks: int
    cout: int
    cin_real: int
    cin_pad: int
    n_pad: int
    nrep: int
    transposed: bool
    wino: Optional[Tensor] = None
    f16: Optional[Tensor] = None
    bf16: Optional[Tensor] = None
    wx4: Optional[Tensor] = None
    exit: Optional[Tensor] = None
    entry: Optional[Tensor] = None
    s2: Optional["PackedWeight"] = None


class LaunchTimer:

    def __init__(self):
        self.records = []

    def summary(self):
        torch.cuda.synchronize()
        out = {}
        for var, flops, e0, e1 in self.records:
            d = out.setdefault(var, {"launches": 0, "ms": 0.0, "flops": 0.0})
            d["launches"] += 1
            d["ms"] += e0.elapsed_time(e1)
            d["flops"] += flops
        return out


_TIMER: Optional[LaunchTimer] = None


def set_launch_timer(t: Optional[LaunchTimer]) -> None:
    global _TIMER
    _TIMER = t


def _timer_start():
    if _TIMER is None:
        return None
    ev = (torch.cuda.Event(enable_timing=True), torch.cuda.Event(enable_timing=True))
    ev[0].record()
    return ev


def _timer_stop(ev, key: tuple, flops: float) -> None:
    ev[1].record()
    _TIMER.records.append((key, flops) + ev)


def _timed_call(fn, args: tuple, what: str, key, flops: float) -> None:
    if _TIMER is None:
        nat.check(fn(*args, nat.stream_handle()), what)
        return
    if callable(key):
        key = key()
    ev = _timer_start()
    nat.check(fn(*args, nat.stream_handle()), what)
    _timer_stop(ev, key, flops)


_CONV_FORMS = {"direct": ("virnet_conv_mfma", "w", "conv_mfma"), "wino": ("virnet_conv_wino", "wino", "conv_wino"),
               "f16x3": ("virnet_conv_f16", "f16", "conv_f16"), "bf16": ("virnet_conv_bf16", "bf16", "conv_bf16"),
               "wx4": ("virnet_conv_wx4", "wx4", "conv_wx4")}


def _conv_key(d: "nat.ConvDesc", form: str, what: str) -> tuple:
    if form != "direct":
        return (form + ("_s2" if d.stride == 2 else "_t" if d.epi == nat.EPI_CONVT else ""), d.cout)
    var = (C.c_int * 4)()
    nat.check(nat.load().virnet_conv_mfma_variant(C.byref(d), C.byref(var)), what)
    return tuple(var)


def _launch_conv(d: "nat.ConvDesc", flops: float, what: str, form: str = "direct", te: Optional["nat.TEmit"] = None) -> None:
    lib = nat.load()
    if te is None:
        fn, args = getattr(lib, _CONV_FORMS[form][0]), (C.byref(d),)
    elif form == "wx4":
        fn, args = lib.virnet_conv_wx4_emit, (C.byref(d), C.byref(te))
    else:
        fn, args = lib.virnet_conv_f16_emit, (C.byref(d), C.byref(te), int(form == "bf16"))
    _timed_call(fn, args, what, lambda: _conv_key(d, form, what), flops)


WINO_MIN_CHANNELS = 32
DEFAULT_CONV_FORM = "wx4"


_KNOBS = ("VIRNET_BIAS_FUSED", "VIRNET_ENTRY_FUSED", "VIRNET_T_EMIT", "VIRNET_WX4_EMIT_ROWS", "VIRNET_WX4_ROWS", "VIRNET_CONV_FORM", "VIRNET_WINOGRAD", "VIRNET_WX4_MIN_COUT", "VIRNET_WX4_MIN_TILES", "VIRNET_WX4_MIN_FILL", "VIRNET_WX4_MIN_WGS", "VIRNET_WX4_MIN_SLAB_WGS",
          "VIRNET_RANGE_GUARD", "VIRNET_WGRAD_FORM", "VIRNET_DETERMINISTIC", "VIRNET_KNET_PERSISTENT", "VIRNET_EXIT_FORM", "VIRNET_SFT_MULTI", "VIRNET_ENTRY_FORM", "VIRNET_GUARD_CHECK", "VIRNET_AUTOGRAPH", "VIRNET_AUTOGRAPH_MAX_PIXELS", "VIRNET_AUTOGRAPH_MAX_GRAPHS")
class forward_scope:

    def __init__(self, form: Optional[str] = None):
        self._form = form

    def __enter__(self):
        tls = nat.tls
        self._prev = (getattr(tls, "scope_env", None), getattr(tls, "stream_cache", None))
        tls.scope_env = {k: os.environ.get(k) for k in _KNOBS}
        self._prev_form = getattr(tls, "form_override", None)
        if self._form is not None:
            tls.form_override = self._form
        if getattr(tls, "form_override", None) is not None:
            tls.scope_env["VIRNET_CONV_FORM"] = tls.form_override
        tls.scope_env["#parsed"] = {}
        tls.stream_cache = torch.cuda.current_stream().cuda_stream if torch.cuda.is_available() else None
        return self

    def __exit__(self, *exc):
        nat.tls.scope_env, nat.tls.stream_cache = self._prev
        nat.tls.form_override = self._prev_form
        return False


def _env(name: str, default=None):
    snap = getattr(nat.tls, "scope_env", None)
    if snap is not None:
        v = snap.get(name)
        return default if v is None else v
    return os.environ.get(name, default)


def _parsed(key: str, make):
    snap = getattr(nat.tls, "scope_env", None)
    if snap is None:
        return make()
    cache = snap["#parsed"]
    v = cache.get(key)
    if v is None:
        v = cache[key] = make()
    return v


def _conv_form_now() -> str:
    form = _env("VIRNET_CONV_FORM")
    if form is None:
        legacy = _env("VIRNET_WINOGRAD")
        form = DEFAULT_CONV_FORM if legacy is None else ("direct" if legacy == "0" else "wino")
    if form not in ("f16x3", "wino", "direct", "bf16", "wx4"):
        raise ValueError(f"VIRNET_CONV_FORM={form!r}: expected wx4, f16x3, wino, direct or bf16")
    return form


def conv_form() -> str:
    return _parsed("form", _conv_form_now)


_F16_FAMILY = ("f16x3", "bf16", "wx4")


def _f16_family() -> bool:
    return conv_form() in _F16_FAMILY


def _wx4_rule():
    return (int(_env("VIRNET_WX4_MIN_COUT", "64")), int(_env("VIRNET_WX4_MIN_TILES", "1")), float(_env("VIRNET_WX4_MIN_FILL", "0.6")),
            _env("VIRNET_DETERMINISTIC", "0") == "1", int(_env("VIRNET_WX4_MIN_WGS", "128")), int(_env("VIRNET_WX4_MIN_SLAB_WGS", "192")))


def wx4_shape_ok(n: int, h: int, w: int, cout: int) -> bool:
    min_cout, min_tiles, min_fill, deterministic, min_wgs, min_slab_wgs = _parsed("wx4_rule", _wx4_rule)
    if cout < min_cout:
        return False
    th, tw = (h + 15) // 16, (w + 31) // 32
    fill = (h * w) / float(th * 16 * tw * 32)
    if th * tw < min_tiles or fill < min_fill:
        return False
    if deterministic:
        return True
    if n * th * tw * ((cout + 95) // 96) >= min_wgs:
        return True
    return cout % 96 == 0 and n * ((h + 7) // 8) * tw * (cout // 32) >= min_slab_wgs


WX4_EMIT_MIN_WGS = 128


def conv_form_rule(has_wino: bool, has_f16: bool, has_bf16: bool, has_wx4: bool, transposed: bool, stride: int, cstore_is_cout: bool,
                   n: int, h: int, w: int, c: int, cout: int, res: bool, mask: bool, mul: bool, in_mul: bool,
                   want_raw: bool, want_act: bool, emit: bool) -> Tuple[str, int]:
    form = "direct"
    plain = not (mask or mul or in_mul)
    if transposed and has_f16 and _f16_family() and plain and want_raw != want_act:
        form = "f16x3"
    elif stride == 2 and not transposed and cstore_is_cout and has_f16 and _f16_family() and not res and plain and not (want_raw and want_act):
        form = "f16x3"
    elif stride == 1 and not transposed and cstore_is_cout:
        want = conv_form()
        if want == "wino" and has_wino:
            form = "wino"
        elif want == "bf16" and has_bf16:
            form = "bf16"
        elif want == "wx4" and has_wx4 and wx4_shape_ok(n, h, w, cout):
            form = "wx4"
        elif want in _F16_FAMILY and has_f16 and cout % 32 == 0:
            form = "f16x3"
    if not (emit and form == "wx4"):
        return form, 0
    unpinned = _env("VIRNET_DETERMINISTIC", "0") != "1" and _env("VIRNET_WX4_MIN_WGS") != "0"
    if has_f16 and (in_mul or c < 32 or (n * ((h + 15) // 16) * ((w + 31) // 32) * ((cout + 95) // 96) < WX4_EMIT_MIN_WGS and unpinned)):
        return "f16x3", 0
    if not t_emission_enabled():
        return form, 0
    return form, 8 if _env("VIRNET_WX4_EMIT_ROWS", "8") == "8" and unpinned and _env("VIRNET_WX4_ROWS") != "16" else 16


def pack_wx4_weight(weight: Tensor, *, dgrad: bool = False) -> Tensor:
    lib = nat.load()
    return _pack_image(weight, dgrad, lib.virnet_wx4_weight_floats, lib.virnet_pack_wx4_weight, "pack_wx4_weight", "Winograd", "virnet_conv_wx4")


def wx4_last_plan() -> dict:
    out = (C.c_int * 4)()
    nat.load().virnet_conv_wx4_last_plan(out)
    return {"rows": out[0], "persistent": bool(out[1]), "slabs": out[2], "launches": out[3]}


def conv_plan_query(family: int, desc: "nat.ConvDesc", *, emit_rows: int = 0, n_cu: int = 0) -> list:
    lib = nat.load()
    out = (nat.ConvLaunch * 4)()
    n = lib.virnet_conv_plan_query(family, C.byref(desc), emit_rows, n_cu, out, 4)
    if n < 0:
        nat.check(n, "conv_plan_query")
    return [{k: getattr(out[i], k) for k, _ in nat.ConvLaunch._fields_} for i in range(n)]


def range_guard_enabled() -> bool:
    return _env("VIRNET_RANGE_GUARD", "1") != "0"


def range_flag(device: torch.device) -> Optional[Tensor]:
    if not range_guard_enabled():
        return None
    idx = device.index if device.index is not None else torch.cuda.current_device()
    flags = getattr(nat.tls, "range_flags", None)
    if flags is None:
        flags = nat.tls.range_flags = {}
    flag = flags.get(idx)
    if flag is None:
        flag = torch.zeros(1, dtype=torch.int32, device=torch.device("cuda", idx))
        with torch.cuda.device(idx):
            nat.check(nat.load().virnet_set_range_flag(nat.ptr(flag)), "set_range_flag")
        flags[idx] = flag
    return flag


def range_overflowed(device: torch.device, *, reset: bool = True) -> bool:
    flag = range_flag(device)
    if flag is None or not bool(flag.item()):
        return False
    if reset:
        flag.zero_()
    return True


def poison_on_flag(flag: Tensor, y: Tensor) -> None:
    nat.check(nat.load().virnet_poison_on_flag(nat.ptr(flag), nat.ptr(y), y.numel(), nat.stream_handle()), "poison_on_flag")


def pack_f16_weight(weight: Tensor, *, dgrad: bool = False, bf16: bool = False) -> Tensor:
    lib = nat.load()
    return _pack_image(weight, dgrad, lib.virnet_f16_weight_floats, lib.virnet_pack_bf16_weight if bf16 else lib.virnet_pack_f16_weight,
                       "pack_f16_weight", "split-fp16")


def pack_wino_weight(weight: Tensor, *, dgrad: bool = False) -> Tensor:
    lib = nat.load()
    return _pack_image(weight, dgrad, lib.virnet_wino_weight_floats, lib.virnet_pack_wino_weight, "pack_wino_weight", "Winograd", "the Winograd kernel")


def _pack_image(weight: Tensor, dgrad: bool, floats, pack, what: str, form: str, whole_blocks: Optional[str] = None) -> Tensor:
    weight = weight.detach()
    _dev_check(weight, "weight")
    cout, cin, kh, kw = weight.shape
    if (kh, kw) != (3, 3):
        raise ValueError(f"the {form} form is for 3x3 kernels")
    rows, ks = (cin, cout) if dgrad else (cout, cin)
    if whole_blocks is not None and rows % 32:
        raise ValueError(f"{whole_blocks} stores multiples of 32 channels, got {rows}")
    n_pad = (rows + 31) // 32 * 32
    cin_pad = (ks + 15) // 16 * 16
    out = torch.empty(floats(cin_pad, n_pad), dtype=torch.float32, device=weight.device)
    nat.check(pack(nat.ptr(weight), int(dgrad), cout, cin, cin_pad, n_pad, nat.ptr(out), nat.stream_handle()), what)
    return out


def _dev_check(t: Tensor, name: str) -> None:
    if not t.is_cuda:
        raise RuntimeError(f"{name} is on {t.device}: the VIRNet HIP path needs tensors on a ROCm device "
                           f"(no CPU fallback exists; move the module and inputs with .cuda())")
    if t.dtype != torch.float32:
        raise TypeError(f"{name} must be float32, got {t.dtype}")
    if not t.is_contiguous():
        raise ValueError(f"{name} must be contiguous")


def get_plan(ks: int, stride: int, cin: int, gemm_n: int) -> nat.ConvPlan:
    plan = nat.ConvPlan()
    nat.check(nat.load().virnet_conv_get_plan(ks, stride, cin, gemm_n, C.byref(plan)), "conv_get_plan")
    return plan


def pack_weight(weight: Tensor, bias: Optional[Tensor], *, transposed: bool = False, stride: int = 1,
                dgrad: bool = False) -> PackedWeight:
    lib = nat.load()
    weight = weight.detach()
    _dev_check(weight, "weight")
    if dgrad:
        if transposed:
            cin, cout, kh, kw = weight.shape
            plan = get_plan(1, 1, 4 * cout, cin)
            kind, ks, gemm_ks = 3, 2, 1
        else:
            cout, cin, kh, kw = weight.shape
            if (kh, kw) != (3, 3):
                raise ValueError("dgrad packing handles 3x3 convs and the 2x2 transposed conv")
            plan = get_plan(3, 1, cout, cin)
            kind, ks, gemm_ks = 2, 3, 3
        n = lib.virnet_packed_weight_floats(gemm_ks, plan.cin_pad, plan.n_pad)
        out = torch.empty(n, dtype=torch.float32, device=weight.device)
        nat.check(lib.virnet_pack_weight(nat.ptr(weight), kind, cout, cin, ks, plan.cin_pad, plan.n_pad, plan.nrep, nat.ptr(out),
                                         nat.stream_handle()), "pack_weight(dgrad)")
        pw = PackedWeight(out, None, gemm_ks, cin, (4 * cout if transposed else cout), plan.cin_pad, plan.n_pad, plan.nrep, False)
        if transposed and _f16_family() and cin % 32 == 0 and cout % 16 == 0:
            k3 = torch.zeros((cin, cout, 3, 3), dtype=torch.float32, device=weight.device)
            k3[:, :, 1:, 1:] = weight
            pw.s2 = pack_weight(k3, None, stride=2)
        if not transposed and cin % 32 == 0 and cout < WINO_MIN_CHANNELS and _f16_family():
            pw.f16 = pack_f16_weight(weight, dgrad=True)
        if not transposed and cin % 32 == 0 and cout >= WINO_MIN_CHANNELS:
            if conv_form() == "wino":
                pw.wino = pack_wino_weight(weight, dgrad=True)
            elif _f16_family():
                pw.f16 = pack_f16_weight(weight, dgrad=True)
                if conv_form() == "bf16":
                    pw.bf16 = pack_f16_weight(weight, dgrad=True, bf16=True)
                if conv_form() == "wx4":
                    pw.wx4 = pack_wx4_weight(weight, dgrad=True)
        return pw
    if transposed:
        cin, cout, kh, kw = weight.shape
        if (kh, kw) != (2, 2):
            raise ValueError("only ConvTranspose2d(k=2, s=2) is on the path (networks/AttResUNet.py:80)")
        plan = get_plan(1, 1, cin, 4 * cout)
        gemm_ks, kind, ks = 1, 1, 2
    else:
        cout, cin, kh, kw = weight.shape
        if kh != kw or kh not in (1, 3):
            raise ValueError(f"unsupported kernel {kh}x{kw}")
        plan = get_plan(kh, stride, cin, cout)
        gemm_ks, kind, ks = kh, 0, kh
    n = lib.virnet_packed_weight_floats(gemm_ks, plan.cin_pad, plan.n_pad)
    out = torch.empty(n, dtype=torch.float32, device=weight.device)
    nat.check(lib.virnet_pack_weight(nat.ptr(weight), kind, cout, cin, ks, plan.cin_pad, plan.n_pad, plan.nrep,
                                     nat.ptr(out), nat.stream_handle()), "pack_weight")
    b = None
    if bias is not None:
        b = bias.detach()
        _dev_check(b, "bias")
    pw = PackedWeight(out, b, gemm_ks, cout, cin, plan.cin_pad, plan.n_pad, plan.nrep, transposed)
    if transposed and _f16_family() and cout % 32 == 0 and cin % 16 == 0:
        pw.f16 = torch.empty(lib.virnet_f16_convt_weight_floats(cin, cout), dtype=torch.float32, device=weight.device)
        nat.check(lib.virnet_pack_f16_convt_weight(nat.ptr(weight), cout, cin, nat.ptr(pw.f16), nat.stream_handle()), "pack_f16_convt_weight")
    if kind == 0 and ks == 3 and stride == 2 and _f16_family() and cout % 32 == 0 and cin % 16 == 0:
        pw.f16 = pack_f16_weight(weight)
    if kind == 0 and ks == 3 and stride == 1:
        if conv_form() == "wino" and cout % 32 == 0 and cin >= WINO_MIN_CHANNELS:
            pw.wino = pack_wino_weight(weight)
        elif _f16_family() and (cout % 32 == 0 or cout <= 32):
            pw.f16 = pack_f16_weight(weight)
            if cin <= 8 and cout % 32 == 0 and cout <= 96:
                pw.entry = torch.empty(lib.virnet_entry_weight_floats(cin, cout), dtype=torch.float32, device=weight.device)
                nat.check(lib.virnet_pack_entry_weight(nat.ptr(weight), cout, cin, cout, nat.ptr(pw.entry), nat.stream_handle()), "pack_entry_weight")
            if cout * 9 <= 32:
                pw.exit = torch.empty(lib.virnet_exit_weight_floats(plan.cin_pad), dtype=torch.float32, device=weight.device)
                nat.check(lib.virnet_pack_exit_weight(nat.ptr(weight), cout, cin, plan.cin_pad, nat.ptr(pw.exit), nat.stream_handle()), "pack_exit_weight")
            if conv_form() == "bf16" and cout % 32 == 0 and cin >= WINO_MIN_CHANNELS:
                pw.bf16 = pack_f16_weight(weight, bf16=True)
            if conv_form() == "wx4" and cout % 32 == 0 and cin >= WINO_MIN_CHANNELS:
                pw.wx4 = pack_wx4_weight(weight)
    return pw


@dataclass
class TImage:
    buf: Tensor
    n: int
    h: int
    w: int
    c: int
    bf16: bool
    db: Optional[Tensor] = None
    pooled: bool = False
    col: Optional[Tensor] = None
    nblk: int = 0
    ncol: int = 0
    col_gen: Optional[Tuple[int, int]] = None

    def col_fresh(self) -> None:
        if self.col is not None and self.col_gen is not None:
            turn, gen = self.col_gen
            now = getattr(nat.tls, "emit_col_gen", {}).get(turn)
            if now != gen:
                raise RuntimeError(f"TImage: the bias-gradient partials of this image were overwritten (workspace {turn}: generation {gen} -> {now}): "
                                   "more than one other emitting convolution ran before its weight gradient consumed them")

    def bias_sums(self) -> Optional[Tensor]:
        self.col_fresh()
        if self.db is None and self.col is not None:
            self.db = _zeros(self.ncol, self.col.device)
            nat.check(nat.load().virnet_colpart_reduce(nat.ptr(self.col), nat.ptr(self.db), self.nblk, self.c // 32, self.ncol, nat.stream_handle()),
                      "colpart_reduce")
            self.col = None
        return self.db


_T_POOL: dict = {}
T_POOL_MAX_BYTES = int(os.environ.get("VIRNET_T_POOL_MB", "8192")) << 20


def _t_pool_trim() -> None:
    total = sum(b.numel() for free in _T_POOL.values() for b in free)
    for key in list(_T_POOL):
        if total <= T_POOL_MAX_BYTES:
            break
        total -= sum(b.numel() for b in _T_POOL[key])
        del _T_POOL[key]


def t_acquire(n: int, h: int, w: int, c: int, bf16: bool, device: torch.device) -> TImage:
    key = (device.index, torch.cuda.current_stream(device).cuda_stream, n, h, w, c)
    free = _T_POOL.get(key)
    buf = free.pop() if free else torch.zeros(nat.load().virnet_chsplit_bytes(n, h, w, c), dtype=torch.uint8, device=device)
    return TImage(buf, n, h, w, c, bf16, None, True)


def t_release(t: Optional[TImage]) -> None:
    if t is not None and t.pooled and t.buf is not None:
        dev = t.buf.device
        key = (dev.index, torch.cuda.current_stream(dev).cuda_stream, t.n, t.h, t.w, t.c)
        free = _T_POOL.pop(key, [])
        free.append(t.buf)
        _T_POOL[key] = free
        t.buf = None
        if len(free) == 1 and len(_T_POOL) > 1:
            _t_pool_trim()


class zero_arena:

    def __init__(self, nfloats: int, device: torch.device):
        self.n, self.device = int(nfloats), device

    def __enter__(self):
        self._prev = getattr(nat.tls, "zero_arena", None)
        nat.tls.zero_arena = [torch.zeros(self.n, dtype=torch.float32, device=self.device), 0] if self.n > 0 else None
        return self

    def __exit__(self, *exc):
        nat.tls.zero_arena = self._prev
        return False


def _zeros(n: int, device: torch.device) -> Tensor:
    ar = getattr(nat.tls, "zero_arena", None)
    if ar is not None and ar[0].device == device and ar[1] + n <= ar[0].numel():
        out = ar[0][ar[1]:ar[1] + n]
        ar[1] += n
        return out
    return torch.zeros(n, dtype=torch.float32, device=device)


def t_pool_clear() -> None:
    _T_POOL.clear()


def t_emission_enabled() -> bool:
    return _env("VIRNET_T_EMIT", "1") != "0"


def conv_mfma(x: Tensor, pw: PackedWeight, *, stride: int = 1, res: Optional[Tensor] = None,
              mul: Optional[Tensor] = None, add: Optional[Tensor] = None, want_raw: bool = True,
              want_act: bool = False, slope: float = 0.2, in_slope: Optional[float] = None,
              in_mul: Optional[Tensor] = None, in_add: Optional[Tensor] = None, mask: Optional[Tensor] = None,
              mask_slope: float = 0.2, out_channels: Optional[int] = None, emit: Optional[dict] = None):
    _dev_check(x, "x")
    n, h, w, c = x.shape
    if c != pw.cin_pad:
        raise ValueError(f"x has {c} channels, packed weight expects {pw.cin_pad}")
    if pw.transposed:
        oh, ow, epi = 2 * h, 2 * w, nat.EPI_CONVT
    else:
        oh, ow, epi = h // stride, w // stride, nat.EPI_NHWC
    cstore = pw.cout if out_channels is None else out_channels
    raw = torch.empty((n, oh, ow, cstore), dtype=torch.float32, device=x.device) if want_raw else None
    act = torch.empty((n, oh, ow, cstore), dtype=torch.float32, device=x.device) if want_act else None
    if mask is not None:
        _dev_check(mask, "mask")
        if tuple(mask.shape) != (n, oh, ow, cstore):
            raise ValueError(f"mask shape {tuple(mask.shape)} != {(n, oh, ow, cstore)}")
    for t, nm in ((res, "res"), (mul, "mul"), (add, "add"), (in_mul, "in_mul"), (in_add, "in_add")):
        if t is not None:
            _dev_check(t, nm)
    if in_mul is not None and (tuple(in_mul.shape) != (n, c) or tuple(in_add.shape) != (n, c)):
        raise ValueError(f"in_mul/in_add must be [{n}, {c}]")
    if res is not None and tuple(res.shape) != (n, oh, ow, cstore):
        raise ValueError(f"res shape {tuple(res.shape)} != {(n, oh, ow, cstore)}")
    form, rows = conv_form_rule(pw.wino is not None, pw.f16 is not None, pw.bf16 is not None, pw.wx4 is not None, pw.transposed, stride,
                                cstore == pw.cout, n, h, w, c, pw.cout, res is not None, mask is not None, mul is not None, in_mul is not None,
                                want_raw, want_act, emit is not None)
    _, image, what = _CONV_FORMS[form]
    wimg = getattr(pw, image)
    d = nat.ConvDesc(x=nat.ptr(x), wpack=nat.ptr(wimg), bias=nat.ptr(pw.bias), res=nat.ptr(res), mul=nat.ptr(mul),
                     add=nat.ptr(add), mask=nat.ptr(mask), mask_slope=mask_slope, in_mul=nat.ptr(in_mul), in_add=nat.ptr(in_add),
                     y_raw=nat.ptr(raw), y_act=nat.ptr(act), n=n, h=h, w=w, cin_pad=c, cout=cstore, n_pad=pw.n_pad, nrep=pw.nrep, ks=pw.ks,
                     stride=stride, epi=epi, nchw_op=0, crop_h=0, crop_w=0, res_sf=1, in_act=int(in_slope is not None),
                     in_slope=0.0 if in_slope is None else in_slope, slope=slope, clamp_lo=0.0, clamp_hi=0.0)
    flops = 2.0 * n * h * w * pw.cin_real * pw.cout * 4 if pw.transposed else 2.0 * n * oh * ow * pw.cin_real * pw.cout * pw.ks ** 2
    if emit is None:
        _launch_conv(d, flops, what, form)
        return raw, act
    timg = None
    nblk = C.c_int(0)
    if (t_emission_enabled() and form in _F16_FAMILY and not pw.transposed and stride == 1
            and nat.load().virnet_conv_emit_ok(C.byref(d), (2 if rows == 8 else 1) if form == "wx4" else 0, C.byref(nblk))):
        timg = t_acquire(n, oh, ow, cstore, form == "bf16", x.device)
        col = None
        ncol = emit.get("colsum")
        if ncol is not None:
            turn = nat.tls.emit_col_turn = getattr(nat.tls, "emit_col_turn", 0) ^ 1
            col = _workspace("emit_col%d" % turn, nblk.value * cstore * 4, x.device)
            gens = getattr(nat.tls, "emit_col_gen", None)
            if gens is None:
                gens = nat.tls.emit_col_gen = {}
            gens[turn] = gens.get(turn, 0) + 1
            timg.col, timg.nblk, timg.ncol, timg.col_gen = col, nblk.value, ncol, (turn, gens[turn])
        slope_t = emit.get("act")
        te = nat.TEmit(t_out=nat.ptr(timg.buf), col=nat.ptr(col), act=int(slope_t is not None), slope=0.0 if slope_t is None else slope_t,
                       bf16=int(form == "bf16"), rows=rows)
        _launch_conv(d, flops, what + "(+T)", form, te)
        if col is not None and _env("VIRNET_BIAS_FUSED", "1") == "0":
            timg.bias_sums()
    else:
        _launch_conv(d, flops, what, form)
    return raw, act, timg


def _planar_out(x: Tensor, pw: PackedWeight, crop_hw: Tuple[int, int], res: Optional[Tensor], res_sf: int, fits: bool, why: str):
    _dev_check(x, "x")
    n, h, w, c = x.shape
    if c != pw.cin_pad or not fits:
        raise ValueError(f"x has {c} channels" + why.format(cin_pad=pw.cin_pad, cout=pw.cout))
    ch, cw = crop_hw
    out = torch.empty((n, pw.cout, ch, cw), dtype=torch.float32, device=x.device)
    if res is not None:
        _dev_check(res, "res")
        if tuple(res.shape) != (n, pw.cout, ch // res_sf, cw // res_sf):
            raise ValueError(f"res shape {tuple(res.shape)} != {(n, pw.cout, ch // res_sf, cw // res_sf)}")
    return n, h, w, c, ch, cw, out


def conv_mfma_nchw(x: Tensor, pw: PackedWeight, crop_hw: Tuple[int, int], *, op: int = nat.NCHW_PLAIN,
                   res: Optional[Tensor] = None, res_sf: int = 1, clamp: Tuple[float, float] = (0.0, 0.0)) -> Tensor:
    n, h, w, c, ch, cw, out = _planar_out(x, pw, crop_hw, res, res_sf, True, ", packed weight expects {cin_pad}")
    d = nat.ConvDesc(x=nat.ptr(x), wpack=nat.ptr(pw.w), bias=nat.ptr(pw.bias), res=nat.ptr(res), mul=0, add=0, mask=0,
                     mask_slope=0.0, in_mul=0, in_add=0, in_act=0, in_slope=0.0, y_raw=nat.ptr(out), y_act=0, n=n, h=h, w=w, cin_pad=c, cout=pw.cout, n_pad=pw.n_pad,
                     nrep=pw.nrep, ks=pw.ks, stride=1, epi=nat.EPI_NCHW, nchw_op=op, crop_h=ch, crop_w=cw,
                     res_sf=res_sf, slope=0.0, clamp_lo=clamp[0], clamp_hi=clamp[1])
    _launch_conv(d, 2.0 * n * h * w * pw.cin_real * pw.cout * pw.ks ** 2, "conv_mfma(nchw)")
    return out


def conv_f16_nchw(x: Tensor, pw: PackedWeight, crop_hw: Tuple[int, int], *, op: int = nat.NCHW_PLAIN,
                  res: Optional[Tensor] = None, res_sf: int = 1, clamp: Tuple[float, float] = (0.0, 0.0)) -> Tensor:
    n, h, w, c, ch, cw, out = _planar_out(x, pw, crop_hw, res, res_sf, pw.f16 is not None and pw.cout <= 32,
                                          " / weight has no split-fp16 image for a planar store (cin_pad {cin_pad}, cout {cout})")
    lib = nat.load()
    use_exit = pw.exit is not None and _env("VIRNET_EXIT_FORM", "rows") != "f16"
    d = nat.ConvDesc(x=nat.ptr(x), wpack=nat.ptr(pw.exit if use_exit else pw.f16), bias=nat.ptr(pw.bias), res=nat.ptr(res), mul=0, add=0, mask=0,
                     mask_slope=0.0, in_mul=0, in_add=0, in_act=0, in_slope=0.0, y_raw=nat.ptr(out), y_act=0, n=n, h=h, w=w, cin_pad=c, cout=pw.cout,
                     n_pad=32, nrep=1, ks=3, stride=1, epi=nat.EPI_NCHW, nchw_op=op, crop_h=ch, crop_w=cw,
                     res_sf=res_sf, slope=0.0, clamp_lo=clamp[0], clamp_hi=clamp[1])
    flops = 2.0 * n * h * w * pw.cin_real * pw.cout * 9
    if use_exit:
        _timed_call(lib.virnet_conv_exit, (C.byref(d),), "conv_exit", ("exit", pw.cout), flops)
    else:
        _timed_call(lib.virnet_conv_f16, (C.byref(d),), "conv_f16(nchw)", ("f16x3", pw.cout), flops)
    return out


def pack_thin_weight(weight: Tensor, bias: Optional[Tensor]) -> PackedWeight:
    lib = nat.load()
    weight = weight.detach()
    _dev_check(weight, "weight")
    cout, cin, kh, kw = weight.shape
    if (kh, kw) != (3, 3) or not 1 <= cout <= 4:
        raise ValueError(f"thin conv handles 3x3 kernels with 1..4 output channels, got {tuple(weight.shape)}")
    c_pad = (cin + 15) // 16 * 16
    out = torch.empty(lib.virnet_thin_weight_floats(c_pad), dtype=torch.float32, device=weight.device)
    nat.check(lib.virnet_pack_thin_weight(nat.ptr(weight), cout, cin, c_pad, nat.ptr(out), nat.stream_handle()), "pack_thin_weight")
    b = None
    if bias is not None:
        b = bias.detach()
        _dev_check(b, "bias")
    return PackedWeight(out, b, 3, cout, cin, c_pad, 4, 0, False)


def conv3x3_thin(x: Tensor, pw: PackedWeight, crop_hw: Tuple[int, int], *, op: int = nat.NCHW_PLAIN,
                 res: Optional[Tensor] = None, res_sf: int = 1, clamp: Tuple[float, float] = (0.0, 0.0)) -> Tensor:
    n, h, w, c, ch, cw, out = _planar_out(x, pw, crop_hw, res, res_sf, pw.nrep == 0, " / weight is not a thin pack (expects {cin_pad})")
    d = nat.ThinDesc(x=nat.ptr(x), wpack=nat.ptr(pw.w), bias=nat.ptr(pw.bias), res=nat.ptr(res), y=nat.ptr(out), n=n, h=h, w=w,
                     c=c, cout=pw.cout, crop_h=ch, crop_w=cw, op=op, res_sf=res_sf, clamp_lo=clamp[0], clamp_hi=clamp[1])
    _timed_call(nat.load().virnet_conv3x3_thin, (C.byref(d),), "conv3x3_thin", ("thin", 3, 1, pw.cout), 2.0 * n * h * w * pw.cin_real * pw.cout * 9)
    return out


def conv_planar(x: Tensor, conv, crop_hw: Tuple[int, int], **kw) -> Tensor:
    if _f16_family() and conv.cout <= 32:
        return conv_f16_nchw(x, conv.packed(), crop_hw, **kw)
    if conv.cout <= 4:
        return conv3x3_thin(x, conv.packed_thin(), crop_hw, **kw)
    return conv_mfma_nchw(x, conv.packed(), crop_hw, **kw)


def pack_input(x: Tensor, hp: int, wp: int, *, sf: int = 1, vec: Optional[Tensor] = None,
               map_: Optional[Tensor] = None, map_sf: int = 1, map_sqrt: bool = False, zero_pad: bool = False) -> Tensor:
    _dev_check(x, "x")
    n, c0, h, w = x.shape
    ev = 0 if vec is None else vec.shape[1]
    em, mh, mw = (0, 0, 0) if map_ is None else map_.shape[1:]
    if vec is not None:
        _dev_check(vec, "vec")
    if map_ is not None:
        _dev_check(map_, "map")
    out = torch.empty((n, hp, wp, 16), dtype=torch.float32, device=x.device)
    d = nat.PackDesc(x=nat.ptr(x), vec=nat.ptr(vec), map=nat.ptr(map_), out=nat.ptr(out), n=n, c0=c0, h=h, w=w, sf=sf,
                     ev=ev, em=em, mh=mh, mw=mw, msf=map_sf, map_sqrt=int(map_sqrt), hp=hp, wp=wp, zero_pad=int(zero_pad))
    nat.check(nat.load().virnet_pack_input(C.byref(d), nat.stream_handle()), "pack_input")
    return out


def conv_entry(x: Tensor, pw: PackedWeight, hp: int, wp: int, *, sf: int = 1, vec: Optional[Tensor] = None, map_: Optional[Tensor] = None,
               map_sf: int = 1, map_sqrt: bool = False, want_act: bool = False, slope: float = 0.2) -> Tensor:
    _dev_check(x, "x")
    n, c0, h, w = x.shape
    ev = 0 if vec is None else vec.shape[1]
    em, mh, mw = (0, 0, 0) if map_ is None else map_.shape[1:]
    kw = dict(want_raw=not want_act, want_act=want_act, slope=slope)
    if not (_f16_family() and pw.f16 is not None and pw.cin_pad == 16 and pw.cout % 32 == 0 and c0 + ev + em <= 8
            and _env("VIRNET_ENTRY_FUSED", "1") != "0"):
        rec = pack_input(x, hp, wp, sf=sf, vec=vec, map_=map_, map_sf=map_sf, map_sqrt=map_sqrt)
        raw, act = conv_mfma(rec, pw, **kw)
        return act if want_act else raw
    for t, nm in ((vec, "vec"), (map_, "map")):
        if t is not None:
            _dev_check(t, nm)
    out = torch.empty((n, hp, wp, pw.cout), dtype=torch.float32, device=x.device)
    use_entry = pw.entry is not None and c0 + ev + em == pw.cin_real and _env("VIRNET_ENTRY_FORM", "rows") != "f16"
    d = nat.ConvDesc(x=nat.ptr(x), wpack=nat.ptr(pw.entry if use_entry else pw.f16), bias=nat.ptr(pw.bias), res=0, mul=0, add=0, mask=0, mask_slope=0.0, in_mul=0, in_add=0,
                     y_raw=0 if want_act else nat.ptr(out), y_act=nat.ptr(out) if want_act else 0, n=n, h=hp, w=wp, cin_pad=16, cout=pw.cout,
                     n_pad=pw.n_pad, nrep=pw.nrep, ks=3, stride=1, epi=nat.EPI_NHWC, nchw_op=0, crop_h=0, crop_w=0, res_sf=1, in_act=0,
                     in_slope=0.0, slope=slope, clamp_lo=0.0, clamp_hi=0.0)
    e = nat.PackDesc(x=nat.ptr(x), vec=nat.ptr(vec), map=nat.ptr(map_), out=0, n=n, c0=c0, h=h, w=w, sf=sf, ev=ev, em=em, mh=mh, mw=mw,
                     msf=map_sf, map_sqrt=int(map_sqrt), hp=hp, wp=wp, zero_pad=0)
    lib = nat.load()
    flops = 2.0 * n * hp * wp * pw.cin_real * pw.cout * 9
    if use_entry:
        _timed_call(lib.virnet_conv_entry, (C.byref(d), C.byref(e)), "conv_entry", ("entry", pw.cout), flops)
    else:
        _timed_call(lib.virnet_conv_f16_entry, (C.byref(d), C.byref(e)), "conv_f16_entry", ("f16x3", pw.cout), flops)
    return out


GAP_MEAN, GAP_EXPCLAMP, GAP_KINFO = nat.GAP_MEAN, nat.GAP_EXPCLAMP, nat.GAP_KINFO


def gap_nchw(x: Tensor, finish: int = GAP_MEAN, clamp: Tuple[float, float] = (0.0, 0.0)) -> Tensor:
    _dev_check(x, "x")
    n, c, h, w = x.shape
    out = torch.empty((n, c), dtype=torch.float32, device=x.device)
    nat.check(nat.load().virnet_gap_nchw(nat.ptr(x), nat.ptr(out), n, c, h, w, finish, clamp[0], clamp[1],
                                         nat.stream_handle()), "gap_nchw")
    return out


def conv_head_s4(x: Tensor, weight: Tensor) -> Tensor:
    _dev_check(x, "x")
    weight = weight.detach()
    _dev_check(weight, "weight")
    n, cin, h, w = x.shape
    cout = weight.shape[0]
    if tuple(weight.shape[1:]) != (cin, 9, 9):
        raise ValueError(f"head weight {tuple(weight.shape)} does not match a 9x9 conv on {cin} channels")
    oh, ow = (h - 1) // 4 + 1, (w - 1) // 4 + 1
    out = torch.empty((n, oh, ow, cout), dtype=torch.float32, device=x.device)
    nat.check(nat.load().virnet_conv_head_s4(nat.ptr(x), nat.ptr(weight), nat.ptr(out), n, cin, h, w, cout,
                                             nat.stream_handle()), "conv_head_s4")
    return out


def conv_head_s4_wgrad(x: Tensor, dy: Tensor, cout: int) -> Tensor:
    _dev_check(x, "x"); _dev_check(dy, "dy")
    n, cin, h, w = x.shape
    oh, ow = (h - 1) // 4 + 1, (w - 1) // 4 + 1
    if tuple(dy.shape) != (n, oh, ow, cout):
        raise ValueError(f"dy shape {tuple(dy.shape)} != {(n, oh, ow, cout)}")
    dw = torch.empty((cout, cin, 9, 9), dtype=torch.float32, device=x.device)
    nat.check(nat.load().virnet_conv_head_s4_wgrad(nat.ptr(x), nat.ptr(dy), nat.ptr(dw), n, cin, h, w, cout, nat.stream_handle()),
              "conv_head_s4_wgrad")
    return dw


def conv_head_s4_dgrad(dy: Tensor, weight: Tensor, hw: Tuple[int, int]) -> Tensor:
    _dev_check(dy, "dy")
    weight = weight.detach()
    _dev_check(weight, "weight")
    n, oh, ow, cout = dy.shape
    h, w = hw
    if tuple(weight.shape[0:1]) != (cout,) or tuple(weight.shape[2:]) != (9, 9) or cout % 4:
        raise ValueError(f"head weight {tuple(weight.shape)} does not match a 9x9 conv to {cout} channels")
    if (oh, ow) != ((h - 1) // 4 + 1, (w - 1) // 4 + 1):
        raise ValueError(f"dy {tuple(dy.shape)} is not the stride-4 output of a {h}x{w} image")
    if weight.device != dy.device:
        raise ValueError(f"weight on {weight.device}, dy on {dy.device}")
    cin = weight.shape[1]
    dx = torch.empty((n, cin, h, w), dtype=torch.float32, device=dy.device)
    nat.check(nat.load().virnet_conv_head_s4_dgrad(nat.ptr(dy), nat.ptr(weight), nat.ptr(dx), n, cin, h, w, cout, nat.stream_handle()),
              "conv_head_s4_dgrad")
    return dx


def image_grad(hw: Tuple[int, int], c0: int, *, n: Optional[int] = None, dres: Optional[Tensor] = None, sf: int = 1,
               ga: Optional[Tensor] = None, wa: Optional[Tensor] = None, gb: Optional[Tensor] = None, wb: Optional[Tensor] = None,
               into: Optional[Tensor] = None) -> Tensor:
    h, w = hw
    srcs = [t for t in (dres, ga, gb, into) if t is not None]
    if n is None:
        if not srcs:
            raise ValueError("image_grad: no term and no batch size")
        n = srcs[0].shape[0]
    for t, nm in ((dres, "dres"), (ga, "ga"), (wa, "wa"), (gb, "gb"), (wb, "wb"), (into, "into")):
        if t is not None:
            _dev_check(t, nm)
    if not 1 <= c0 <= 4 or sf < 1:
        raise ValueError(f"image_grad: c0={c0} (1..4), sf={sf}")
    dev = srcs[0].device if srcs else None
    if any(t.device != dev for t in srcs + [t for t in (wa, wb) if t is not None]):
        raise ValueError("image_grad: tensors on different devices")
    if dres is not None and tuple(dres.shape) != (n, c0, h * sf, w * sf):
        raise ValueError(f"image_grad: dres {tuple(dres.shape)} != {(n, c0, h * sf, w * sf)}")
    hp = wp = ca = cina = cb = cinb = 0
    if ga is not None:
        if wa is None:
            raise ValueError("image_grad: ga without wa")
        _, hp, wp, ca = ga.shape
        if ga.shape[0] != n or tuple(wa.shape[::2]) != (ca, 3) or wa.shape[3] != 3 or wa.shape[1] < c0 or ca % 4:
            raise ValueError(f"image_grad: ga {tuple(ga.shape)} / wa {tuple(wa.shape)} do not match")
        cina = wa.shape[1]
    if gb is not None:
        if wb is None:
            raise ValueError("image_grad: gb without wb")
        cb = gb.shape[3]
        if tuple(gb.shape[:3]) != (n, h, w) or tuple(wb.shape[::2]) != (cb, 3) or wb.shape[3] != 3 or wb.shape[1] < c0 or cb % 4:
            raise ValueError(f"image_grad: gb {tuple(gb.shape)} / wb {tuple(wb.shape)} do not match {(n, h, w)}")
        cinb = wb.shape[1]
    if into is not None and tuple(into.shape) != (n, c0, h, w):
        raise ValueError(f"image_grad: into {tuple(into.shape)} != {(n, c0, h, w)}")
    out = into if into is not None else torch.empty((n, c0, h, w), dtype=torch.float32, device=dev)
    d = nat.ImageGradDesc(dres=nat.ptr(dres), ga=nat.ptr(ga), wa=nat.ptr(wa), gb=nat.ptr(gb), wb=nat.ptr(wb), dx=nat.ptr(out),
                          n=n, c0=c0, h=h, w=w, sf=sf, hp=hp, wp=wp, ca=ca, cina=cina, cb=cb, cinb=cinb, accumulate=int(into is not None))
    nat.check(nat.load().virnet_image_grad(C.byref(d), nat.stream_handle()), "image_grad")
    return out


def ca_gate(x: Tensor, w1: Tensor, b1: Tensor, w2: Tensor, b2: Tensor) -> Tensor:
    _dev_check(x, "x")
    n, h, w, c = x.shape
    cr = w1.shape[0]
    ts = [t.detach() for t in (w1, b1, w2, b2)]
    for t in ts:
        _dev_check(t, "CALayer parameter")
    gate = torch.empty((n, c), dtype=torch.float32, device=x.device)
    nat.check(nat.load().virnet_ca_gate(nat.ptr(x), *(nat.ptr(t) for t in ts), nat.ptr(gate), n, h, w, c, cr,
                                        nat.stream_handle()), "ca_gate")
    return gate


CA_FUSED_MAX_ITEMS = 16 * 1024


def ca_scale_add(hcv: Tensor, w1: Tensor, b1: Tensor, w2: Tensor, b2: Tensor, skip: Tensor) -> Tensor:
    _dev_check(hcv, "hcv"); _dev_check(skip, "skip")
    n, h, w, c = hcv.shape
    if h * w * (c // 4) > CA_FUSED_MAX_ITEMS or c % 4 or 256 % c:
        return scale_add(hcv, ca_gate(hcv, w1, b1, w2, b2), skip)
    ts = [t.detach() for t in (w1, b1, w2, b2)]
    for t in ts:
        _dev_check(t, "CALayer parameter")
    out = torch.empty_like(hcv)
    nat.check(nat.load().virnet_ca_scale_add(nat.ptr(hcv), *(nat.ptr(t) for t in ts), nat.ptr(skip), nat.ptr(out), n, h, w, c, w1.shape[0],
                                             nat.stream_handle()), "ca_scale_add")
    return out


KNET_BODY_MAX = 16


def knet_body(x: Tensor, layers) -> Tensor:
    _dev_check(x, "x")
    n, h, w, c = x.shape
    arr = (nat.KnetLayer * len(layers))()
    keep = []
    for i, (p1, p2, w1, b1, w2, b2) in enumerate(layers):
        if p1.f16 is None or p2.f16 is None:
            raise RuntimeError("knet_body needs the split-fp16 weight images (VIRNET_CONV_FORM of the f16 family)")
        ts = [t.detach() for t in (w1, b1, w2, b2)]
        for t in ts:
            _dev_check(t, "CALayer parameter")
        keep.append(ts)
        arr[i] = nat.KnetLayer(nat.ptr(p1.f16), 0 if p1.bias is None else nat.ptr(p1.bias), nat.ptr(p2.f16), 0 if p2.bias is None else nat.ptr(p2.bias),
                               *(nat.ptr(t) for t in ts))
    out = torch.empty_like(x)
    cr = layers[0][2].shape[0]
    nat.check(nat.load().virnet_knet_body(nat.ptr(x), nat.ptr(out), C.cast(arr, C.c_void_p), len(layers), n, h, w, c, cr, nat.stream_handle()),
              "knet_body")
    return out


def scale_add(hcv: Tensor, gate: Tensor, skip: Tensor) -> Tensor:
    _dev_check(hcv, "hcv"); _dev_check(skip, "skip"); _dev_check(gate, "gate")
    n, h, w, c = hcv.shape
    out = torch.empty_like(hcv)
    nat.check(nat.load().virnet_scale_add(nat.ptr(hcv), nat.ptr(gate), nat.ptr(skip), nat.ptr(out), n, h * w, c,
                                          nat.stream_handle()), "scale_add")
    return out


def _sft_weights(att) -> Tuple[nat.SftWeights, list]:
    c1, c2, cm, ca = att.conv1, att.conv2, att.mul_conv, att.add_conv
    ps = (c1.weight, c1.bias, c2.weight, c2.bias, cm.weight, cm.bias, ca.weight, ca.bias)
    key = tuple((p.data_ptr(), p._version) for p in ps)
    hit = att.__dict__.get("_sftw")
    if hit is not None and hit[0] == key:
        return hit[1], hit[2]
    ts = [p.detach() for p in ps]
    for t in ts:
        _dev_check(t, "AttLayer parameter")
    wt = nat.SftWeights(*(nat.ptr(t) for t in ts), e=c1.cin, nf1=c1.cout, nf2=c2.cout, nf=cm.cout)
    att.__dict__["_sftw"] = (key, wt, ts)
    return wt, ts


def sft_vec(vec: Tensor, att) -> Tuple[Tensor, Tensor]:
    _dev_check(vec, "vec")
    n = vec.shape[0]
    wt, keep = _sft_weights(att)
    if vec.shape[1] != wt.e:
        raise ValueError(f"conditioning vector has {vec.shape[1]} channels, AttLayer expects {wt.e}")
    mul = torch.empty((n, wt.nf), dtype=torch.float32, device=vec.device)
    add = torch.empty_like(mul)
    nat.check(nat.load().virnet_sft_vec(nat.ptr(vec), C.byref(wt), nat.ptr(mul), nat.ptr(add), n, nat.stream_handle()),
              "sft_vec")
    return mul, add


SFT_MULTI_MAX = 16


def sft_vec_multi(vec: Tensor, atts) -> list:
    _dev_check(vec, "vec")
    n = vec.shape[0]
    out = []
    lib = nat.load()
    for i0 in range(0, len(atts), SFT_MULTI_MAX):
        group = atts[i0:i0 + SFT_MULTI_MAX]
        wts = (nat.SftWeights * len(group))()
        muls, adds = (C.c_void_p * len(group))(), (C.c_void_p * len(group))()
        keep = []
        for l, att in enumerate(group):
            wt, ts = _sft_weights(att)
            if vec.shape[1] != wt.e:
                raise ValueError(f"conditioning vector has {vec.shape[1]} channels, AttLayer expects {wt.e}")
            keep.append(ts)
            wts[l] = wt
            mul = torch.empty((n, wt.nf), dtype=torch.float32, device=vec.device)
            add = torch.empty_like(mul)
            muls[l], adds[l] = nat.ptr(mul), nat.ptr(add)
            out.append((mul, add))
        nat.check(lib.virnet_sft_vec_multi(nat.ptr(vec), wts, len(group), muls, adds, n, nat.stream_handle()), "sft_vec_multi")
    return out


def sft_apply(raw: Tensor, rec: Tensor, chan0: int, nchan: int, step: int, att) -> Tensor:
    _dev_check(raw, "raw"); _dev_check(rec, "rec")
    n, h, w, nf = raw.shape
    wt, keep = _sft_weights(att)
    if nchan != wt.e or nf != wt.nf:
        raise ValueError(f"AttLayer({wt.e}->{wt.nf}) does not match conditioning {nchan} / features {nf}")
    if tuple(rec.shape) != (n, h * step, w * step, 16):
        raise ValueError(f"rec shape {tuple(rec.shape)} != {(n, h * step, w * step, 16)}")
    act = torch.empty_like(raw)
    nat.check(nat.load().virnet_sft_apply(nat.ptr(raw), nat.ptr(rec), C.byref(wt), nat.ptr(act), n, h, w, step, chan0,
                                          nat.stream_handle()), "sft_apply")
    return act


def conv_wgrad(x: Tensor, dy: Tensor, weight_shape: Tuple[int, ...], *, stride: int = 1, transposed: bool = False,
               in_slope: Optional[float] = None, in_mul: Optional[Tensor] = None, in_add: Optional[Tensor] = None,
               bias_channels: Optional[int] = None, xt: Optional[TImage] = None, yt: Optional[TImage] = None):
    _dev_check(x, "x"); _dev_check(dy, "dy")
    n, h, w, cx = x.shape
    cy = dy.shape[3]
    if transposed:
        cin, cout, ks = weight_shape[0], weight_shape[1], 1
    else:
        cout, cin, ks = weight_shape[0], weight_shape[1], weight_shape[2]
    form = conv_form()
    if not transposed and stride == 1 and ks == 3 and h >= 5 and _f16_family() and _env("VIRNET_WGRAD_FORM", "f16") != "f32":
        dw = torch.empty(weight_shape, dtype=torch.float32, device=x.device)
        bf = form == "bf16" and (min(cin, cout) >= 32 or (xt is not None and xt.bf16) or (yt is not None and yt.bf16))
        return _conv_wgrad_f16(x, dy, dw, cin, cout, in_slope, in_mul, in_add, bf16=bf, bias_channels=bias_channels, xt=xt, yt=yt)
    if not transposed and stride == 2 and ks == 3 and _wgrad_s2_ok(h // 2, cx):
        return _conv_wgrad_f16_s2(x, dy, weight_shape, 0, in_slope, in_mul, in_add, bf16=(form == "bf16" and min(cin, cout) >= 32),
                                  bias_channels=bias_channels, lo_t=yt)
    dw = torch.zeros(weight_shape, dtype=torch.float32, device=x.device)
    rows = 4 * cout if transposed else cout
    ctr = torch.zeros(((rows + 31) // 32) * ((cin + 31) // 32), dtype=torch.int32, device=x.device)
    d = nat.WgradDesc(x=nat.ptr(x), dy=nat.ptr(dy), in_mul=nat.ptr(in_mul), in_add=nat.ptr(in_add), dw=nat.ptr(dw),
                      counters=nat.ptr(ctr), n=n, h=h, w=w,
                      cx=cx, cy=cy, cin=cin, cout=cout, ks=ks, stride=stride, transposed=int(transposed),
                      in_act=int(in_slope is not None), in_slope=0.0 if in_slope is None else in_slope)
    pix = n * (h // stride) * (w // stride)
    _timed_call(nat.load().virnet_conv_wgrad, (C.byref(d),), "conv_wgrad", ("wgrad", ks, stride, int(transposed)),
                2.0 * pix * cin * cout * (4 if transposed else ks * ks))
    if bias_channels is not None:
        return dw, colsum(dy, bias_channels)
    return dw


def convt_dgrad(dy: Tensor, pw: PackedWeight) -> Tensor:
    if pw.s2 is not None and pw.s2.f16 is not None and _f16_family():
        return conv_mfma(dy, pw.s2, stride=2, want_raw=True)[0]
    return conv_mfma(space_to_depth2(dy), pw, want_raw=True)[0]


def _wgrad_s2_ok(oh: int, chi: int) -> bool:
    return _f16_family() and _env("VIRNET_WGRAD_FORM", "f16") != "f32" and oh >= 5 and chi % 32 == 0


def convt_wgrad(x: Tensor, dy: Tensor, weight_shape: Tuple[int, ...], xt: Optional[TImage] = None):
    _dev_check(x, "x"); _dev_check(dy, "dy")
    n, h, w, cx = x.shape
    cin, cout = weight_shape[0], weight_shape[1]
    if tuple(dy.shape) != (n, 2 * h, 2 * w, cout):
        raise ValueError(f"dy shape {tuple(dy.shape)} != {(n, 2 * h, 2 * w, cout)}")
    if _wgrad_s2_ok(h, cout):
        return _conv_wgrad_f16_s2(dy, x, weight_shape, 1, None, None, None, bf16=(conv_form() == "bf16" and min(cin, cout) >= 32),
                                  bias_channels=cout, lo_t=xt)
    return conv_wgrad(x, space_to_depth2(dy), weight_shape, transposed=True), colsum(dy)


def conv_wgrad_plan_query(n: int, h: int, w: int, cx: int, cy: int, mode: int = 0) -> dict:
    out = nat.WgradF16Plan()
    nat.check(nat.load().virnet_conv_wgrad_f16_plan_query(n, h, w, cx, cy, mode, C.byref(out)), "conv_wgrad_f16_plan_query")
    return {k: getattr(out, k) for k, _ in nat.WgradF16Plan._fields_}


_WORKSPACES: dict = {}


def _workspace(tag: str, nbytes: int, device: torch.device) -> Tensor:
    key = (device.index, torch.cuda.current_stream(device).cuda_stream, tag)
    buf = _WORKSPACES.get(key)
    if buf is None or buf.numel() < nbytes:
        buf = torch.empty(int(nbytes * 1.25) if buf is not None else nbytes, dtype=torch.uint8, device=device)
        _WORKSPACES[key] = buf
    return buf


def _conv_wgrad_f16(x: Tensor, dy: Tensor, dw: Tensor, cin: int, cout: int, in_slope, in_mul, in_add, *, bf16: bool,
                    bias_channels: Optional[int] = None, xt: Optional[TImage] = None, yt: Optional[TImage] = None):
    lib = nat.load()
    n, h, w, cx = x.shape
    cy = dy.shape[3]
    st = nat.stream_handle()
    for t, cc, nm in ((xt, cx, "xt"), (yt, cy, "yt")):
        if t is not None and ((t.n, t.h, t.w, t.c) != (n, h, w, cc) or t.buf is None):
            raise ValueError(f"conv_wgrad: {nm} is a T image of {(t.n, t.h, t.w, t.c)}, expected {(n, h, w, cc)}")
    if xt is not None and xt.bf16 != bf16:
        xt = None
    if yt is not None and yt.bf16 != bf16:
        yt = None
    if yt is not None and bias_channels is not None and not ((yt.db is not None and yt.db.numel() == bias_channels)
                                                             or (yt.col is not None and yt.ncol == bias_channels)):
        yt = None
    ev = _timer_start()
    if xt is None:
        xbuf = _workspace("wgrad_xt", lib.virnet_chsplit_bytes(n, h, w, cx), x.device)
        nat.check(lib.virnet_chsplit(nat.ptr(x), n, h, w, cx, int(in_slope is not None), 0.0 if in_slope is None else in_slope,
                                     nat.ptr(in_mul), nat.ptr(in_add), int(bf16), nat.ptr(xbuf), None, None, 0, st), "chsplit")
    else:
        xbuf = xt.buf
    db = col = None
    if yt is None:
        ybuf = _workspace("wgrad_yt", lib.virnet_chsplit_bytes(n, h, w, cy), x.device)
        if bias_channels is not None:
            db = _zeros(bias_channels, x.device)
            col = _workspace("wgrad_col", lib.virnet_chsplit_colsum_bytes(n, h, w, cy), x.device)
        nat.check(lib.virnet_chsplit(nat.ptr(dy), n, h, w, cy, 0, 0.0, None, None, int(bf16), nat.ptr(ybuf), nat.ptr(col), nat.ptr(db),
                                     0 if bias_channels is None else bias_channels, st), "chsplit")
    else:
        ybuf = yt.buf
        db = yt.db if bias_channels is not None else None
    pending = yt is not None and bias_channels is not None and db is None
    scr = _workspace("wgrad_part", lib.virnet_conv_wgrad_f16_scratch_bytes(n, h, w, cx, cy), x.device)
    if pending:
        yt.col_fresh()
        db = _zeros(bias_channels, x.device)
        nat.check(lib.virnet_conv_wgrad_f16_db(nat.ptr(xbuf), nat.ptr(ybuf), nat.ptr(dw), nat.ptr(scr), n, h, w, cx, cy, cin, cout, int(bf16),
                                               nat.ptr(yt.col), nat.ptr(db), yt.nblk, bias_channels, st), "conv_wgrad_f16_db")
        yt.db, yt.col = db, None
    else:
        nat.check(lib.virnet_conv_wgrad_f16(nat.ptr(xbuf), nat.ptr(ybuf), nat.ptr(dw), nat.ptr(scr), n, h, w, cx, cy, cin, cout, int(bf16), st), "conv_wgrad_f16")
    if ev is not None:
        _timer_stop(ev, ("wgrad_f16", 3, 1, 0), 2.0 * n * h * w * cin * cout * 9)
    return dw if bias_channels is None else (dw, db)


def _conv_wgrad_f16_s2(hi: Tensor, lo: Tensor, weight_shape, mode: int, in_slope, in_mul, in_add, *, bf16: bool,
                       bias_channels: Optional[int] = None, lo_t: Optional[TImage] = None):
    lib = nat.load()
    n, hh, hw, chi = hi.shape
    _, oh, ow, clo = lo.shape
    if (hh, hw) != (2 * oh, 2 * ow):
        raise ValueError(f"stride-2 weight gradient: {tuple(hi.shape)} is not twice {tuple(lo.shape)}")
    st = nat.stream_handle()
    if lo_t is not None and ((lo_t.n, lo_t.h, lo_t.w, lo_t.c) != (n, oh, ow, clo) or lo_t.bf16 != bf16 or lo_t.buf is None
                             or (mode == 0 and bias_channels is not None and (lo_t.ncol if lo_t.db is None else lo_t.db.numel()) != bias_channels)):
        lo_t = None
    ht = _workspace("wgrad_xt", lib.virnet_chsplit_s2_bytes(n, hh, hw, chi), hi.device)
    lt = lo_t.buf if lo_t is not None else _workspace("wgrad_yt", lib.virnet_chsplit_bytes(n, oh, ow, clo), hi.device)
    ev = _timer_start()
    db = None
    hcol = lcol = None
    if bias_channels is not None:
        db = _zeros(bias_channels, hi.device)
        if mode == 1:
            hcol = _workspace("wgrad_col", lib.virnet_chsplit_s2_colsum_bytes(n, hh, hw, chi), hi.device)
        elif lo_t is not None:
            db = lo_t.bias_sums()
        else:
            lcol = _workspace("wgrad_col", lib.virnet_chsplit_colsum_bytes(n, oh, ow, clo), hi.device)
    bc = 0 if bias_channels is None else bias_channels
    nat.check(lib.virnet_chsplit_s2(nat.ptr(hi), n, hh, hw, chi, int(in_slope is not None), 0.0 if in_slope is None else in_slope,
                                    nat.ptr(in_mul), nat.ptr(in_add), int(bf16), nat.ptr(ht), nat.ptr(hcol), nat.ptr(db) if hcol is not None else None,
                                    bc if hcol is not None else 0, st), "chsplit_s2")
    if lo_t is None:
        nat.check(lib.virnet_chsplit(nat.ptr(lo), n, oh, ow, clo, 0, 0.0, None, None, int(bf16), nat.ptr(lt), nat.ptr(lcol),
                                     nat.ptr(db) if lcol is not None else None, bc if lcol is not None else 0, st), "chsplit")
    if mode == 0:
        cout, cin = weight_shape[0], weight_shape[1]
    else:
        cin, cout = weight_shape[0], weight_shape[1]
    dw = torch.empty(weight_shape, dtype=torch.float32, device=hi.device)
    scr = _workspace("wgrad_part", lib.virnet_conv_wgrad_f16_s2_scratch_bytes(n, oh, ow, chi, clo), hi.device)
    nat.check(lib.virnet_conv_wgrad_f16_s2(nat.ptr(ht), nat.ptr(lt), nat.ptr(dw), nat.ptr(scr), n, oh, ow, chi, clo, cin, cout, mode, int(bf16), st),
              "conv_wgrad_f16_s2")
    if ev is not None:
        _timer_stop(ev, ("wgrad_f16_s2", 3 if mode == 0 else 2, 2, mode), 2.0 * n * oh * ow * cin * cout * (4 if mode else 9))
    return dw if bias_channels is None else (dw, db)


def colsum(dy: Tensor, cvalid: Optional[int] = None) -> Tensor:
    _dev_check(dy, "dy")
    c = dy.shape[-1]
    cvalid = c if cvalid is None else cvalid
    db = _zeros(cvalid, dy.device)
    nat.check(nat.load().virnet_colsum(nat.ptr(dy), nat.ptr(db), dy.numel() // c, c, cvalid, nat.stream_handle()), "colsum")
    return db


def sft_backward(da: Tensor, x: Tensor, mul: Tensor, add: Tensor, *, slope: float = 0.2, res: Optional[Tensor] = None):
    for t, nm in ((da, "da"), (x, "x"), (mul, "mul"), (add, "add")):
        _dev_check(t, nm)
    n, h, w, c = x.shape
    if tuple(da.shape) != (n, h, w, c) or tuple(mul.shape) != (n, c) or tuple(add.shape) != (n, c):
        raise ValueError(f"sft_backward: da {tuple(da.shape)} / mul {tuple(mul.shape)} / add {tuple(add.shape)} do not match x {tuple(x.shape)}")
    if res is not None:
        _dev_check(res, "res")
        if tuple(res.shape) != (n, h, w, c):
            raise ValueError(f"sft_backward: res {tuple(res.shape)} != {(n, h, w, c)}")
    dx = torch.empty_like(x)
    dmul = torch.zeros((n, c), dtype=torch.float32, device=x.device)
    dadd = torch.zeros((n, c), dtype=torch.float32, device=x.device)
    nat.check(nat.load().virnet_sft_backward(nat.ptr(da), nat.ptr(x), nat.ptr(mul), nat.ptr(add), nat.ptr(res), slope, nat.ptr(dx), nat.ptr(dmul),
                                             nat.ptr(dadd), n, h * w, c, nat.stream_handle()), "sft_backward")
    return dx, dmul, dadd


def zero_stuff2(dy: Tensor) -> Tensor:
    _dev_check(dy, "dy")
    n, h, w, c = dy.shape
    z = torch.empty((n, 2 * h, 2 * w, c), dtype=torch.float32, device=dy.device)
    nat.check(nat.load().virnet_zero_stuff2(nat.ptr(dy), nat.ptr(z), n, h, w, c, nat.stream_handle()), "zero_stuff2")
    return z


def space_to_depth2(dy: Tensor) -> Tensor:
    _dev_check(dy, "dy")
    n, h2, w2, c = dy.shape
    out = torch.empty((n, h2 // 2, w2 // 2, 4 * c), dtype=torch.float32, device=dy.device)
    nat.check(nat.load().virnet_space_to_depth2(nat.ptr(dy), nat.ptr(out), n, h2 // 2, w2 // 2, c, nat.stream_handle()), "space_to_depth2")
    return out


def pack_input_backward(drec: Tensor, chan: int, hw: Tuple[int, int], *, map_: Optional[Tensor] = None, map_sqrt: bool = False,
                        into: Optional[Tensor] = None) -> Tensor:
    _dev_check(drec, "drec")
    n, hp, wp, crec = drec.shape
    h, w = hw
    out = into if into is not None else torch.empty((n, 1, h, w), dtype=torch.float32, device=drec.device)
    nat.check(nat.load().virnet_pack_input_backward(nat.ptr(drec), crec, chan, nat.ptr(map_), nat.ptr(out), n, h, w, hp, wp,
                                                    int(map_sqrt), int(into is not None), nat.stream_handle()), "pack_input_backward")
    return out
```

Measured before the change: 1568.

## Compose last resblock conv2 with exit conv into a precomputed tap-map

```diff
diff --git a/include/virnet_hip.h b/include/virnet_hip.h
--- a/include/virnet_hip.h
+++ b/include/virnet_hip.h
@@ -88,6 +88,9 @@
 size_t virnet_exit_weight_floats(int cin_pad);
 int virnet_pack_exit_weight(const float* w_oihw, int cout, int cin, int cin_pad, float* packed, void* stream);
 int virnet_conv_exit(const virnet_conv_desc* d, void* stream);
+int virnet_conv_exit_add(const virnet_conv_desc* d, const float* z_add, void* stream);
+int virnet_compose_exit_weight(const float* w2, const float* b2, const float* w_exit, int cout_exit, int cmid, int cin, float* wc, float* bc,
+                               void* stream);
 
 int virnet_set_range_flag(int* device_flag);
 int virnet_poison_on_flag(const int* device_flag, float* y, size_t n, void* stream);
diff --git a/virnet_amd/_native.py b/virnet_amd/_native.py
--- a/virnet_amd/_native.py
+++ b/virnet_amd/_native.py
@@ -119,6 +119,8 @@
     ("virnet_exit_weight_floats", C.c_size_t, [C.c_int]),
     ("virnet_pack_exit_weight", C.c_int, [C.c_void_p, C.c_int, C.c_int, C.c_int, C.c_void_p, C.c_void_p]),
     ("virnet_conv_exit", C.c_int, [C.POINTER(ConvDesc), C.c_void_p]),
+    ("virnet_conv_exit_add", C.c_int, [C.POINTER(ConvDesc), C.c_void_p, C.c_void_p]),
+    ("virnet_compose_exit_weight", C.c_int, [C.c_void_p, C.c_void_p, C.c_void_p, C.c_int, C.c_int, C.c_int, C.c_void_p, C.c_void_p, C.c_void_p]),
     ("virnet_set_range_flag", C.c_int, [C.c_void_p]),
     ("virnet_poison_on_flag", C.c_int, [C.c_void_p, C.c_void_p, C.c_size_t, C.c_void_p]),
     ("virnet_pack_bf16_weight", C.c_int, [C.c_void_p, C.c_int, C.c_int, C.c_int, C.c_int, C.c_int, C.c_void_p, C.c_void_p]),
diff --git a/virnet_amd/csrc/conv_exit.hip b/virnet_amd/csrc/conv_exit.hip
--- a/virnet_amd/csrc/conv_exit.hip
+++ b/virnet_amd/csrc/conv_exit.hip
@@ -11,166 +11,16 @@
 
 template <int NCH>
 __global__ __launch_bounds__(256) void conv_exit_kernel(const FArgs a) {
-  extern __shared__ __attribute__((aligned(16))) char smem[];
-  const int nch = NCH ? NCH : (a.Cin >> 4);
-  char* const a_lds = smem;
-  float* const z_lds = reinterpret_cast<float*>(smem + nch * 2048);
+  constexpr bool ZADD = false;
+  [[maybe_unused]] const float* const zadd = nullptr;
+#include "conv_exit_body.inc"
+}
 
-  const int xcd = blockIdx.x & 7, q = blockIdx.x >> 3;
-  const int tile = xcd * a.tiles_per_xcd + q;
-  if (q >= a.tiles_per_xcd || tile >= a.ntiles) return;
-  const int img = fast_div(tile, a.mg_tpi);
-  const int trem = tile - img * (a.ntx * a.nty);
-  const int ty = fast_div(trem, a.mg_ntx), tx = trem - ty * a.ntx;
-  const int oy0 = ty * EX_TH, ox0 = tx * EX_TW;
-
-  const int tid = threadIdx.x, lane = tid & 63, wave = __builtin_amdgcn_readfirstlane(tid >> 6);
-  const int l31 = lane & 31, lhi = lane >> 5;
-  const int nrows = a.cout * 9;
-  TSTAMP(0);
-
-  if constexpr (NCH != 0) {
-    f32x4 wv[NCH / 2];
-#pragma unroll
-    for (int i = 0; i < NCH / 2; ++i) wv[i] = *reinterpret_cast<const f32x4*>(a.wimg + i * 4096 + tid * 16);
-#pragma unroll
-    for (int i = 0; i < NCH / 2; ++i) *reinterpret_cast<f32x4*>(a_lds + i * 4096 + tid * 16) = wv[i];
-  } else {
-    for (int i = tid * 16; i < nch * 2048; i += 256 * 16) *reinterpret_cast<f32x4*>(a_lds + i) = *reinterpret_cast<const f32x4*>(a.wimg + i);
-  }
-  __syncthreads();
-  TSTAMP(1);
-
-  const int oyl = tid >> 5, oxl = tid & 31;
-  const int oy = oy0 + oyl, ox = ox0 + oxl;
-  const bool inside = oy < a.crop_h && ox < a.crop_w;
-  const size_t plane = (size_t)a.crop_h * a.crop_w;
-  const size_t o0 = (size_t)img * a.cout * plane + (size_t)oy * a.crop_w + ox;
-  float scv[27], bsv[3];
-#pragma unroll
-  for (int i = 0; i < 27; ++i) scv[i] = a.inv_scale[i];
-#pragma unroll
-  for (int c = 0; c < 3; ++c) bsv[c] = (a.bias && c < a.cout) ? a.bias[c] : 0.f;
-  float rv[3] = {0.f, 0.f, 0.f};
-  if (a.nchw_op == VIRNET_NCHW_ADD && inside) {
-    const int rw = a.crop_w / a.res_sf;
-    const size_t rplane = (size_t)(a.crop_h / a.res_sf) * rw;
-    const size_t r0 = (size_t)img * a.cout * rplane + (size_t)(oy / a.res_sf) * rw + ox / a.res_sf;
-#pragma unroll
-    for (int c = 0; c < 3; ++c)
-      if (c < a.cout) rv[c] = a.res[a.res_sf > 1 ? r0 + c * rplane : o0 + c * plane];
-  }
-
-  const float* const ximg = a.x + (size_t)img * a.H * a.W * a.Cin;
-  float amax = 0.f;
-  auto pixel_of = [&](int blk) -> const float* {
-    const int p = blk * 32 + l31;
-    const int hy = p / EX_HW, hx = p - hy * EX_HW;
-    const int gy = oy0 - 1 + hy, gx = ox0 - 1 + hx;
-    const bool valid = blk < EX_BLK && p < EX_HPX && (unsigned)gy < (unsigned)a.H && (unsigned)gx < (unsigned)a.W;
-    return valid ? ximg + ((size_t)gy * a.W + gx) * a.Cin + lhi * 8 : nullptr;
-  };
-  auto mma = [&](f32x16& acc, int c, f32x4 v0, f32x4 v1) {
-    if (a.in_act) { v0 = lrelu4(v0, a.in_slope); v1 = lrelu4(v1, a.in_slope); }
-    range_note(amax, v0, v1);
-    h8 bh, bl;
-    split8(v0, v1, bh, bl);
-    const h8 ah = *reinterpret_cast<const h8*>(a_lds + c * 2048 + lane * 16);
-    const h8 al = *reinterpret_cast<const h8*>(a_lds + c * 2048 + 1024 + lane * 16);
-    acc = __builtin_amdgcn_mfma_f32_32x32x16_f16(al, bh, acc, 0, 0, 0);
-    acc = __builtin_amdgcn_mfma_f32_32x32x16_f16(ah, bl, acc, 0, 0, 0);
-    acc = __builtin_amdgcn_mfma_f32_32x32x16_f16(ah, bh, acc, 0, 0, 0);
-  };
-  auto put_z = [&](int blk, const f32x16& acc) {
-    const int p = blk * 32 + l31;
-#pragma unroll
-    for (int r = 0; r < 16; ++r) {
-      const int row = 8 * (r >> 2) + 4 * lhi + (r & 3);
-      z_lds[min(row, nrows) * EX_ZS + p] = acc[r];
-    }
-  };
-  if constexpr (NCH != 0) {
-    const auto xrs = __builtin_amdgcn_make_buffer_rsrc(const_cast<float*>(ximg), 0, a.H * a.W * a.Cin * 4, 0x00020000);
-    auto pixel_off = [&](int blk) -> unsigned {
-      const int p = blk * 32 + l31;
-      const int hy = p / EX_HW, hx = p - hy * EX_HW;
-      const int gy = oy0 - 1 + hy, gx = ox0 - 1 + hx;
-      const bool valid = p < EX_HPX && (unsigned)gy < (unsigned)a.H && (unsigned)gx < (unsigned)a.W;
-      return valid ? (unsigned)(((gy * a.W + gx) * a.Cin + lhi * 8) * 4) : 0x80000000u;
-    };
-    auto request = [&](unsigned off, f32x4 (&v0)[NCH], f32x4 (&v1)[NCH]) {
-#pragma unroll
-      for (int c = 0; c < NCH; ++c) {
-        v0[c] = __builtin_bit_cast(f32x4, __builtin_amdgcn_raw_buffer_load_b128(xrs, off + c * 64, 0, 0));
-        v1[c] = __builtin_bit_cast(f32x4, __builtin_amdgcn_raw_buffer_load_b128(xrs, off + c * 64 + 16, 0, 0));
-      }
-    };
-    auto compute = [&](int blk, f32x4 (&v0)[NCH], f32x4 (&v1)[NCH]) {
-      f32x16 acc;
-#pragma unroll
-      for (int r = 0; r < 16; ++r) acc[r] = 0.f;
-#pragma unroll
-      for (int c = 0; c < NCH; ++c) mma(acc, c, v0[c], v1[c]);
-      put_z(blk, acc);
-    };
-    static_assert(EX_BLK > 8 && EX_BLK <= 12, "three blocks per wave at most, two at least");
-    f32x4 p0[NCH], p1[NCH], q0[NCH], q1[NCH];
-    const bool third = wave + 8 < EX_BLK;
-    request(pixel_off(wave), p0, p1);
-    request(pixel_off(wave + 4), q0, q1);
-    compute(wave, p0, p1);
-    if (third) request(pixel_off(wave + 8), p0, p1);
-    compute(wave + 4, q0, q1);
-    if (third) compute(wave + 8, p0, p1);
-  } else {
-    for (int blk = wave; blk < EX_BLK; blk += 4) {
-      const float* const px = pixel_of(blk);
-      f32x16 acc;
-#pragma unroll
-      for (int r = 0; r < 16; ++r) acc[r] = 0.f;
-      for (int c = 0; c < nch; ++c) {
-        f32x4 v0 = f32x4{0.f, 0.f, 0.f, 0.f}, v1 = v0;
-        if (px) {
-          v0 = *reinterpret_cast<const f32x4*>(px + c * 16);
-          v1 = *reinterpret_cast<const f32x4*>(px + c * 16 + 4);
-        }
-        mma(acc, c, v0, v1);
-      }
-      put_z(blk, acc);
-    }
-  }
-  TSTAMP(2);
-  range_report(a.range_flag, amax);
-  __syncthreads();
-  TSTAMP(3);
-#ifdef VIRNET_F16_TIMING
-  if (a.tlog && tid == 0) {
-    a.tlog[(size_t)blockIdx.x * 8 + 5] = __builtin_amdgcn_s_getreg((31 << 11) | (0 << 6) | 4);
-    a.tlog[(size_t)blockIdx.x * 8 + 6] = __builtin_amdgcn_s_getreg((31 << 11) | (0 << 6) | 20);
-  }
-#endif
-
-  if (!inside) return;
-  float outv[3];
-#pragma unroll
-  for (int c = 0; c < 3; ++c) {
-    float v = bsv[c];
-    const float* const zc = z_lds + (c < a.cout ? c * 9 : 0) * EX_ZS + oyl * EX_HW + oxl;
-#pragma unroll
-    for (int dy = 0; dy < 3; ++dy)
-#pragma unroll
-      for (int dx = 0; dx < 3; ++dx) v += zc[(dy * 3 + dx) * EX_ZS + dy * EX_HW + dx] * scv[c * 9 + dy * 3 + dx];
-    if (a.nchw_op == VIRNET_NCHW_ADD) v += rv[c];
-    else if (a.nchw_op == VIRNET_NCHW_EXPCLAMP) v = expf(fminf(fmaxf(v, a.clamp_lo), a.clamp_hi));
-    outv[c] = v;
-  }
-#pragma unroll
-  for (int c = 0; c < 3; ++c)
-    if (c < a.cout) a.y_raw[o0 + c * plane] = outv[c];
-#ifdef VIRNET_F16_TIMING
-  asm volatile("s_waitcnt vmcnt(0)" ::: "memory");
-#endif
-  TSTAMP(4);
+template <int NCH>
+__global__ __launch_bounds__(256) void conv_exit_zadd_kernel(const FArgs a, const float* __restrict__ zadd) {
+  static_assert(NCH != 0, "the additive map rides on the buffer loads of the fixed-count forms");
+  constexpr bool ZADD = true;
+#include "conv_exit_body.inc"
 }
 
 __global__ void pack_exit_kernel(const float* __restrict__ w, int cout, int cin, int cin_pad, float* __restrict__ inv_scale, char* __restrict__ img) {
@@ -219,6 +69,19 @@
   return virnet::check_launch("conv_exit launch");
 }
 
+template <int NCH>
+int launch_exit_zadd(FArgs k, const float* zadd, hipStream_t st) {
+  const int lds = NCH * 2048 + (k.cout * 9 + 1) * EX_ZS * 4;
+  static unsigned long long attr_done = 0;
+  auto kern = conv_exit_zadd_kernel<NCH>;
+  if (virnet::first_use_on_device(attr_done)) {
+    hipError_t e = hipFuncSetAttribute(reinterpret_cast<const void*>(kern), hipFuncAttributeMaxDynamicSharedMemorySize, 160 * 1024);
+    if (e != hipSuccess) return virnet::set_error("hipFuncSetAttribute(conv_exit, z_add): %s", hipGetErrorString(e));
+  }
+  hipLaunchKernelGGL(kern, dim3((unsigned)(8 * k.tiles_per_xcd)), dim3(256), lds, st, k, zadd);
+  return virnet::check_launch("conv_exit(z_add) launch");
+}
+
 #ifdef VIRNET_F16_TIMING
 long long* g_xlog = nullptr;
 #endif
@@ -239,7 +102,7 @@
   return virnet::check_launch("pack_exit launch");
 }
 
-extern "C" int virnet_conv_exit(const virnet_conv_desc* d, void* stream) {
+static int conv_exit_host(const virnet_conv_desc* d, const float* z_add, bool with_z, void* stream) {
   VIRNET_REQUIRE(d != nullptr, "virnet_conv_exit: desc is NULL");
   VIRNET_REQUIRE(d->x && d->wpack && d->y_raw, "virnet_conv_exit: x / wpack / y_raw is NULL");
   VIRNET_REQUIRE(d->ks == 3 && d->stride == 1 && d->epi == VIRNET_EPI_NCHW, "virnet_conv_exit: only the stride-1 3x3 conv with planar store (ks=%d stride=%d epi=%d)",
@@ -271,8 +134,18 @@
   k.mg_tpi = div_magic(k.ntx * k.nty);
   hipStream_t st = static_cast<hipStream_t>(stream);
   const int nch = d->cin_pad >> 4;
+  if (with_z) {
+    VIRNET_REQUIRE(z_add != nullptr, "virnet_conv_exit_add: z_add is NULL");
+    VIRNET_REQUIRE(nch == 6 || nch == 4, "virnet_conv_exit_add: cin_pad=%d (the additive map is built for 96 and 64 input channels)", d->cin_pad);
+    VIRNET_REQUIRE(!d->in_act, "virnet_conv_exit_add: no input activation (z_add is linear in x only without one)");
+    return nch == 6 ? launch_exit_zadd<6>(k, z_add, st) : launch_exit_zadd<4>(k, z_add, st);
+  }
   if (nch == 6) return launch_exit<6>(k, st);
   if (nch == 4) return launch_exit<4>(k, st);
   VIRNET_REQUIRE(nch * 2048 + 33 * EX_ZS * 4 <= 160 * 1024, "virnet_conv_exit: cin_pad=%d does not fit LDS", d->cin_pad);
   return launch_exit<0>(k, st);
 }
+
+extern "C" int virnet_conv_exit(const virnet_conv_desc* d, void* stream) { return conv_exit_host(d, nullptr, false, stream); }
+
+extern "C" int virnet_conv_exit_add(const virnet_conv_desc* d, const float* z_add, void* stream) { return conv_exit_host(d, z_add, true, stream); }
diff --git a/virnet_amd/csrc/conv_exit_body.inc b/virnet_amd/csrc/conv_exit_body.inc
--- /dev/null
+++ b/virnet_amd/csrc/conv_exit_body.inc
@@ -0,0 +1,201 @@
+  extern __shared__ __attribute__((aligned(16))) char smem[];
+  const int nch = NCH ? NCH : (a.Cin >> 4);
+  char* const a_lds = smem;
+  float* const z_lds = reinterpret_cast<float*>(smem + nch * 2048);
+
+  const int xcd = blockIdx.x & 7, q = blockIdx.x >> 3;
+  const int tile = xcd * a.tiles_per_xcd + q;
+  if (q >= a.tiles_per_xcd || tile >= a.ntiles) return;
+  const int img = fast_div(tile, a.mg_tpi);
+  const int trem = tile - img * (a.ntx * a.nty);
+  const int ty = fast_div(trem, a.mg_ntx), tx = trem - ty * a.ntx;
+  const int oy0 = ty * EX_TH, ox0 = tx * EX_TW;
+
+  const int tid = threadIdx.x, lane = tid & 63, wave = __builtin_amdgcn_readfirstlane(tid >> 6);
+  const int l31 = lane & 31, lhi = lane >> 5;
+  const int nrows = a.cout * 9;
+  TSTAMP(0);
+
+  if constexpr (NCH != 0) {
+    f32x4 wv[NCH / 2];
+#pragma unroll
+    for (int i = 0; i < NCH / 2; ++i) wv[i] = *reinterpret_cast<const f32x4*>(a.wimg + i * 4096 + tid * 16);
+#pragma unroll
+    for (int i = 0; i < NCH / 2; ++i) *reinterpret_cast<f32x4*>(a_lds + i * 4096 + tid * 16) = wv[i];
+  } else {
+    for (int i = tid * 16; i < nch * 2048; i += 256 * 16) *reinterpret_cast<f32x4*>(a_lds + i) = *reinterpret_cast<const f32x4*>(a.wimg + i);
+  }
+  __syncthreads();
+  TSTAMP(1);
+
+  const int oyl = tid >> 5, oxl = tid & 31;
+  const int oy = oy0 + oyl, ox = ox0 + oxl;
+  const bool inside = oy < a.crop_h && ox < a.crop_w;
+  const size_t plane = (size_t)a.crop_h * a.crop_w;
+  const size_t o0 = (size_t)img * a.cout * plane + (size_t)oy * a.crop_w + ox;
+  float scv[27], bsv[3];
+#pragma unroll
+  for (int i = 0; i < 27; ++i) scv[i] = a.inv_scale[i];
+#pragma unroll
+  for (int c = 0; c < 3; ++c) bsv[c] = (a.bias && c < a.cout) ? a.bias[c] : 0.f;
+  [[maybe_unused]] float zsc[16];
+  if constexpr (ZADD) {
+#pragma unroll
+    for (int j = 0; j < 4; ++j) {
+      const f32x4 s4 = *reinterpret_cast<const f32x4*>(a.inv_scale + 8 * j + 4 * lhi);
+#pragma unroll
+      for (int i = 0; i < 4; ++i) zsc[4 * j + i] = __builtin_bit_cast(float, 0x7f000000 - __builtin_bit_cast(int, s4[i]));
+    }
+  }
+  float rv[3] = {0.f, 0.f, 0.f};
+  if (a.nchw_op == VIRNET_NCHW_ADD && inside) {
+    const int rw = a.crop_w / a.res_sf;
+    const size_t rplane = (size_t)(a.crop_h / a.res_sf) * rw;
+    const size_t r0 = (size_t)img * a.cout * rplane + (size_t)(oy / a.res_sf) * rw + ox / a.res_sf;
+#pragma unroll
+    for (int c = 0; c < 3; ++c)
+      if (c < a.cout) rv[c] = a.res[a.res_sf > 1 ? r0 + c * rplane : o0 + c * plane];
+  }
+
+  const float* const ximg = a.x + (size_t)img * a.H * a.W * a.Cin;
+  float amax = 0.f;
+  auto pixel_of = [&](int blk) -> const float* {
+    const int p = blk * 32 + l31;
+    const int hy = p / EX_HW, hx = p - hy * EX_HW;
+    const int gy = oy0 - 1 + hy, gx = ox0 - 1 + hx;
+    const bool valid = blk < EX_BLK && p < EX_HPX && (unsigned)gy < (unsigned)a.H && (unsigned)gx < (unsigned)a.W;
+    return valid ? ximg + ((size_t)gy * a.W + gx) * a.Cin + lhi * 8 : nullptr;
+  };
+  auto mma = [&](f32x16& acc, int c, f32x4 v0, f32x4 v1) {
+    if (a.in_act) { v0 = lrelu4(v0, a.in_slope); v1 = lrelu4(v1, a.in_slope); }
+    range_note(amax, v0, v1);
+    h8 bh, bl;
+    split8(v0, v1, bh, bl);
+    const h8 ah = *reinterpret_cast<const h8*>(a_lds + c * 2048 + lane * 16);
+    const h8 al = *reinterpret_cast<const h8*>(a_lds + c * 2048 + 1024 + lane * 16);
+    acc = __builtin_amdgcn_mfma_f32_32x32x16_f16(al, bh, acc, 0, 0, 0);
+    acc = __builtin_amdgcn_mfma_f32_32x32x16_f16(ah, bl, acc, 0, 0, 0);
+    acc = __builtin_amdgcn_mfma_f32_32x32x16_f16(ah, bh, acc, 0, 0, 0);
+  };
+  auto put_z = [&](int blk, const f32x16& acc) {
+    const int p = blk * 32 + l31;
+#pragma unroll
+    for (int r = 0; r < 16; ++r) {
+      const int row = 8 * (r >> 2) + 4 * lhi + (r & 3);
+      z_lds[min(row, nrows) * EX_ZS + p] = acc[r];
+    }
+  };
+  if constexpr (NCH != 0) {
+    const auto xrs = __builtin_amdgcn_make_buffer_rsrc(const_cast<float*>(ximg), 0, a.H * a.W * a.Cin * 4, 0x00020000);
+    auto pixel_off = [&](int blk) -> unsigned {
+      const int p = blk * 32 + l31;
+      const int hy = p / EX_HW, hx = p - hy * EX_HW;
+      const int gy = oy0 - 1 + hy, gx = ox0 - 1 + hx;
+      const bool valid = p < EX_HPX && (unsigned)gy < (unsigned)a.H && (unsigned)gx < (unsigned)a.W;
+      return valid ? (unsigned)(((gy * a.W + gx) * a.Cin + lhi * 8) * 4) : 0x80000000u;
+    };
+    auto request = [&](unsigned off, f32x4 (&v0)[NCH], f32x4 (&v1)[NCH]) {
+#pragma unroll
+      for (int c = 0; c < NCH; ++c) {
+        v0[c] = __builtin_bit_cast(f32x4, __builtin_amdgcn_raw_buffer_load_b128(xrs, off + c * 64, 0, 0));
+        v1[c] = __builtin_bit_cast(f32x4, __builtin_amdgcn_raw_buffer_load_b128(xrs, off + c * 64 + 16, 0, 0));
+      }
+    };
+    auto compute = [&](int blk, f32x4 (&v0)[NCH], f32x4 (&v1)[NCH]) {
+      f32x16 acc;
+#pragma unroll
+      for (int r = 0; r < 16; ++r) acc[r] = 0.f;
+#pragma unroll
+      for (int c = 0; c < NCH; ++c) mma(acc, c, v0[c], v1[c]);
+      put_z(blk, acc);
+    };
+    static_assert(EX_BLK > 8 && EX_BLK <= 12, "three blocks per wave at most, two at least");
+    f32x4 p0[NCH], p1[NCH], q0[NCH], q1[NCH];
+    const bool third = wave + 8 < EX_BLK;
+    if constexpr (!ZADD) {
+      request(pixel_off(wave), p0, p1);
+      request(pixel_off(wave + 4), q0, q1);
+      compute(wave, p0, p1);
+      if (third) request(pixel_off(wave + 8), p0, p1);
+      compute(wave + 4, q0, q1);
+      if (third) compute(wave + 8, p0, p1);
+    } else {
+      const auto zrs = __builtin_amdgcn_make_buffer_rsrc(const_cast<float*>(zadd + (size_t)img * a.H * a.W * 32), 0, a.H * a.W * 128, 0x00020000);
+      auto zadd_off = [&](int blk) -> unsigned {
+        const int p = blk * 32 + l31;
+        const int hy = p / EX_HW, hx = p - hy * EX_HW;
+        const int gy = oy0 - 1 + hy, gx = ox0 - 1 + hx;
+        const bool valid = p < EX_HPX && (unsigned)gy < (unsigned)a.H && (unsigned)gx < (unsigned)a.W;
+        return valid ? (unsigned)(((gy * a.W + gx) * 32 + lhi * 4) * 4) : 0x80000000u;
+      };
+      auto request_z = [&](unsigned off, f32x4 (&z)[4]) {
+#pragma unroll
+        for (int j = 0; j < 4; ++j) z[j] = __builtin_bit_cast(f32x4, __builtin_amdgcn_raw_buffer_load_b128(zrs, off + j * 32, 0, 0));
+      };
+      auto compute_z = [&](int blk, f32x4 (&v0)[NCH], f32x4 (&v1)[NCH], const f32x4 (&z)[4]) {
+        f32x16 acc;
+#pragma unroll
+        for (int r = 0; r < 16; ++r) acc[r] = z[r >> 2][r & 3] * zsc[r];
+#pragma unroll
+        for (int c = 0; c < NCH; ++c) mma(acc, c, v0[c], v1[c]);
+        put_z(blk, acc);
+      };
+      f32x4 zp[4], zq[4];
+      request(pixel_off(wave), p0, p1);
+      request_z(zadd_off(wave), zp);
+      request(pixel_off(wave + 4), q0, q1);
+      request_z(zadd_off(wave + 4), zq);
+      compute_z(wave, p0, p1, zp);
+      if (third) { request(pixel_off(wave + 8), p0, p1); request_z(zadd_off(wave + 8), zp); }
+      compute_z(wave + 4, q0, q1, zq);
+      if (third) compute_z(wave + 8, p0, p1, zp);
+    }
+  } else {
+    for (int blk = wave; blk < EX_BLK; blk += 4) {
+      const float* const px = pixel_of(blk);
+      f32x16 acc;
+#pragma unroll
+      for (int r = 0; r < 16; ++r) acc[r] = 0.f;
+      for (int c = 0; c < nch; ++c) {
+        f32x4 v0 = f32x4{0.f, 0.f, 0.f, 0.f}, v1 = v0;
+        if (px) {
+          v0 = *reinterpret_cast<const f32x4*>(px + c * 16);
+          v1 = *reinterpret_cast<const f32x4*>(px + c * 16 + 4);
+        }
+        mma(acc, c, v0, v1);
+      }
+      put_z(blk, acc);
+    }
+  }
+  TSTAMP(2);
+  range_report(a.range_flag, amax);
+  __syncthreads();
+  TSTAMP(3);
+#ifdef VIRNET_F16_TIMING
+  if (a.tlog && tid == 0) {
+    a.tlog[(size_t)blockIdx.x * 8 + 5] = __builtin_amdgcn_s_getreg((31 << 11) | (0 << 6) | 4);
+    a.tlog[(size_t)blockIdx.x * 8 + 6] = __builtin_amdgcn_s_getreg((31 << 11) | (0 << 6) | 20);
+  }
+#endif
+
+  if (!inside) return;
+  float outv[3];
+#pragma unroll
+  for (int c = 0; c < 3; ++c) {
+    float v = bsv[c];
+    const float* const zc = z_lds + (c < a.cout ? c * 9 : 0) * EX_ZS + oyl * EX_HW + oxl;
+#pragma unroll
+    for (int dy = 0; dy < 3; ++dy)
+#pragma unroll
+      for (int dx = 0; dx < 3; ++dx) v += zc[(dy * 3 + dx) * EX_ZS + dy * EX_HW + dx] * scv[c * 9 + dy * 3 + dx];
+    if (a.nchw_op == VIRNET_NCHW_ADD) v += rv[c];
+    else if (a.nchw_op == VIRNET_NCHW_EXPCLAMP) v = expf(fminf(fmaxf(v, a.clamp_lo), a.clamp_hi));
+    outv[c] = v;
+  }
+#pragma unroll
+  for (int c = 0; c < 3; ++c)
+    if (c < a.cout) a.y_raw[o0 + c * plane] = outv[c];
+#ifdef VIRNET_F16_TIMING
+  asm volatile("s_waitcnt vmcnt(0)" ::: "memory");
+#endif
+  TSTAMP(4);
diff --git a/virnet_amd/csrc/pack.hip b/virnet_amd/csrc/pack.hip
--- a/virnet_amd/csrc/pack.hip
+++ b/virnet_amd/csrc/pack.hip
@@ -109,6 +109,25 @@
   }
 }
 
+__global__ void compose_exit_kernel(const float* __restrict__ w2, const float* __restrict__ b2, const float* __restrict__ we, int ce, int cm,
+                                    int ci, float* __restrict__ wc, float* __restrict__ bc) {
+  const int per_row = ci * 9, total = 32 * per_row;
+  for (int i = blockIdx.x * blockDim.x + threadIdx.x; i < total + 32; i += gridDim.x * blockDim.x) {
+    const bool is_bias = i >= total;
+    const int row = is_bias ? i - total : i / per_row;
+    const int rem = is_bias ? 0 : i - row * per_row;
+    double acc = 0.0;
+    if (row < ce * 9 && !(is_bias && !b2)) {
+      const int c = row / 9, t = row - c * 9;
+      const float* const arow = we + (size_t)c * cm * 9 + t;
+      for (int m = 0; m < cm; ++m)
+        acc += (double)arow[(size_t)m * 9] * (double)(is_bias ? b2[m] : w2[(size_t)m * per_row + rem]);
+    }
+    if (is_bias) bc[row] = (float)acc;
+    else wc[i] = (float)acc;
+  }
+}
+
 }
 
 static int grid_for(size_t total) { return (int)((total + 255) / 256 > 8192 ? 8192 : (total + 255) / 256); }
@@ -181,3 +200,14 @@
   hipLaunchKernelGGL(pack_input_kernel, dim3(grid), dim3(256), 0, static_cast<hipStream_t>(stream), *d);
   return virnet::check_launch("pack_input launch");
 }
+
+extern "C" int virnet_compose_exit_weight(const float* w2, const float* b2, const float* w_exit, int cout_exit, int cmid, int cin, float* wc,
+                                          float* bc, void* stream) {
+  VIRNET_REQUIRE(w2 && w_exit && wc && bc, "virnet_compose_exit_weight: NULL pointer");
+  VIRNET_REQUIRE(cout_exit >= 1 && cout_exit * 9 <= 32, "virnet_compose_exit_weight: cout_exit=%d: the (channel, tap) rows must fit one 32-row block", cout_exit);
+  VIRNET_REQUIRE(cmid >= 1 && cin >= 1 && (long)cin * 9 * 32 < (1L << 30), "virnet_compose_exit_weight: bad extents cmid=%d cin=%d", cmid, cin);
+  const int total = 32 * cin * 9 + 32;
+  hipLaunchKernelGGL(compose_exit_kernel, dim3((total + 255) / 256), dim3(256), 0, static_cast<hipStream_t>(stream), w2, b2, w_exit, cout_exit,
+                     cmid, cin, wc, bc);
+  return virnet::check_launch("compose_exit launch");
+}
diff --git a/virnet_amd/engine.py b/virnet_amd/engine.py
--- a/virnet_amd/engine.py
+++ b/virnet_amd/engine.py
@@ -92,6 +92,35 @@
         f1a = ops.sft_apply(f1, cond.rec, cond.chan0, cond.nchan, 1 << level, blk.sft2)
     out, _ = ops.conv_mfma(f1a, c2, res=x_raw, want_raw=True)
     return out
+
+
+TAIL_COMPOSE_DEFAULT = "1"
+TAIL_COMPOSE_FORM_DEFAULT = "wx4"
+
+
+def _param_key(*params) -> tuple:
+    return tuple(None if p is None else (id(p), p.data_ptr(), p._version, p.device) for p in params)
+
+
+def _tail_composition(rnet) -> Optional[ops.PackedWeight]:
+    if (not ops._f16_family() or ops._env("VIRNET_TAIL_COMPOSE", TAIL_COMPOSE_DEFAULT) == "0" or ops._env("VIRNET_EXIT_FORM", "rows") == "f16"
+            or torch.is_grad_enabled() or len(rnet.up_path) == 0 or len(rnet.up_path[-1].body) == 0):
+        return None
+    blk, tail = rnet.up_path[-1].body[-1], rnet.tail
+    if blk.extra_chn > 0 or tail.ks != 3 or tail.cout * 9 > 32 or blk.nf not in (64, 96) or tail.cin != blk.nf:
+        return None
+    form = ops.conv_form()
+    key = _param_key(blk.conv2.weight, blk.conv2.bias, tail.weight)
+    packs = rnet.__dict__.setdefault("_tail_packs", {})
+    hit = packs.get(form)
+    if hit is None or hit[0] != key:
+        if torch.cuda.is_current_stream_capturing():
+            return None
+        hit = (key, ops.compose_exit_weight(blk.conv2.weight, blk.conv2.bias, tail.weight))
+        for f in [f for f, h in packs.items() if h[0] != key]:
+            del packs[f]
+        packs[form] = hit
+    return hit[1]
 
 
 def rnet_forward(rnet, x_in: Tensor, *, extra_map: Optional[Tensor] = None, extra_vec: Optional[Tensor] = None,
@@ -140,11 +169,18 @@
         if ii + 1 < len(rnet.down_path):
             bridges.append(x)
             x, _ = ops.conv_mfma(x, lvl.downsampler.packed(), stride=2, want_raw=True)
+    composed = _tail_composition(rnet)
     for jj, up in enumerate(rnet.up_path):
         x, _ = ops.conv_mfma(x, up.upsampler.packed(), res=bridges[-jj - 1], want_raw=True)
-        for blk in up.body:
+        last = composed is not None and jj + 1 == len(rnet.up_path)
+        for blk in (up.body[:-1] if last else up.body):
             x = _res_block(x, blk, None, 0)
-    return ops.conv_planar(x, rnet.tail, (H, W), op=nat.NCHW_ADD, res=x_in, res_sf=sf)
+    if composed is None:
+        return ops.conv_planar(x, rnet.tail, (H, W), op=nat.NCHW_ADD, res=x_in, res_sf=sf)
+    blk = rnet.up_path[-1].body[-1]
+    _, t = ops.conv_mfma(x, blk.conv1.packed(), in_slope=0.2, want_raw=False, want_act=True, slope=0.2)
+    z_c, _ = ops.conv_mfma(t, composed, want_raw=True, thin_wx4=ops._env("VIRNET_TAIL_COMPOSE_FORM", TAIL_COMPOSE_FORM_DEFAULT) != "f16x3")
+    return ops.conv_f16_nchw(x, rnet.tail.packed(), (H, W), op=nat.NCHW_ADD, res=x_in, res_sf=sf, z_add=z_c)
 
 
 FP32_FORM = "wino"
diff --git a/virnet_amd/networks/AttResUNet.py b/virnet_amd/networks/AttResUNet.py
--- a/virnet_amd/networks/AttResUNet.py
+++ b/virnet_amd/networks/AttResUNet.py
@@ -79,5 +79,8 @@
             self.up_path.append(UpBlock(n_feat[jj + 1], n_feat[jj], n_resblocks))
         self.tail = ConvParam(n_feat[0], out_chn, 3)
 
+    def invalidate(self) -> None:
+        self.__dict__.pop("_tail_packs", None)
+
     def forward(self, x_in: torch.Tensor, extra_maps_in: Optional[torch.Tensor]) -> torch.Tensor:
         return engine.rnet_forward(self, x_in, extra_map=extra_maps_in)
diff --git a/virnet_amd/ops.py b/virnet_amd/ops.py
--- a/virnet_amd/ops.py
+++ b/virnet_amd/ops.py
@@ -109,7 +109,8 @@
 
 
 _KNOBS = ("VIRNET_BIAS_FUSED", "VIRNET_ENTRY_FUSED", "VIRNET_T_EMIT", "VIRNET_WX4_EMIT_ROWS", "VIRNET_WX4_ROWS", "VIRNET_CONV_FORM", "VIRNET_WINOGRAD", "VIRNET_WX4_MIN_COUT", "VIRNET_WX4_MIN_TILES", "VIRNET_WX4_MIN_FILL", "VIRNET_WX4_MIN_WGS", "VIRNET_WX4_MIN_SLAB_WGS",
-          "VIRNET_RANGE_GUARD", "VIRNET_WGRAD_FORM", "VIRNET_DETERMINISTIC", "VIRNET_KNET_PERSISTENT", "VIRNET_EXIT_FORM", "VIRNET_SFT_MULTI", "VIRNET_ENTRY_FORM", "VIRNET_GUARD_CHECK", "VIRNET_AUTOGRAPH", "VIRNET_AUTOGRAPH_MAX_PIXELS", "VIRNET_AUTOGRAPH_MAX_GRAPHS")
+          "VIRNET_RANGE_GUARD", "VIRNET_WGRAD_FORM", "VIRNET_DETERMINISTIC", "VIRNET_KNET_PERSISTENT", "VIRNET_EXIT_FORM", "VIRNET_SFT_MULTI", "VIRNET_ENTRY_FORM", "VIRNET_GUARD_CHECK", "VIRNET_AUTOGRAPH", "VIRNET_AUTOGRAPH_MAX_PIXELS", "VIRNET_AUTOGRAPH_MAX_GRAPHS",
+          "VIRNET_TAIL_COMPOSE", "VIRNET_TAIL_COMPOSE_FORM")
 class forward_scope:
 
     def __init__(self, form: Optional[str] = None):
@@ -504,7 +505,7 @@
               mul: Optional[Tensor] = None, add: Optional[Tensor] = None, want_raw: bool = True,
               want_act: bool = False, slope: float = 0.2, in_slope: Optional[float] = None,
               in_mul: Optional[Tensor] = None, in_add: Optional[Tensor] = None, mask: Optional[Tensor] = None,
-              mask_slope: float = 0.2, out_channels: Optional[int] = None, emit: Optional[dict] = None):
+              mask_slope: float = 0.2, out_channels: Optional[int] = None, emit: Optional[dict] = None, thin_wx4: bool = False):
     _dev_check(x, "x")
     n, h, w, c = x.shape
     if c != pw.cin_pad:
@@ -530,6 +531,8 @@
     form, rows = conv_form_rule(pw.wino is not None, pw.f16 is not None, pw.bf16 is not None, pw.wx4 is not None, pw.transposed, stride,
                                 cstore == pw.cout, n, h, w, c, pw.cout, res is not None, mask is not None, mul is not None, in_mul is not None,
                                 want_raw, want_act, emit is not None)
+    if thin_wx4 and form == "f16x3" and emit is None and pw.wx4 is not None and conv_form() == "wx4" and wx4_shape_ok(n, h, w, max(pw.cout, 64)):
+        form = "wx4"
     _, image, what = _CONV_FORMS[form]
     wimg = getattr(pw, image)
     d = nat.ConvDesc(x=nat.ptr(x), wpack=nat.ptr(wimg), bias=nat.ptr(pw.bias), res=nat.ptr(res), mul=nat.ptr(mul),
@@ -593,7 +596,7 @@
 
 
 def conv_f16_nchw(x: Tensor, pw: PackedWeight, crop_hw: Tuple[int, int], *, op: int = nat.NCHW_PLAIN,
-                  res: Optional[Tensor] = None, res_sf: int = 1, clamp: Tuple[float, float] = (0.0, 0.0)) -> Tensor:
+                  res: Optional[Tensor] = None, res_sf: int = 1, clamp: Tuple[float, float] = (0.0, 0.0), z_add: Optional[Tensor] = None) -> Tensor:
     n, h, w, c, ch, cw, out = _planar_out(x, pw, crop_hw, res, res_sf, pw.f16 is not None and pw.cout <= 32,
                                           " / weight has no split-fp16 image for a planar store (cin_pad {cin_pad}, cout {cout})")
     lib = nat.load()
@@ -603,11 +606,35 @@
                      n_pad=32, nrep=1, ks=3, stride=1, epi=nat.EPI_NCHW, nchw_op=op, crop_h=ch, crop_w=cw,
                      res_sf=res_sf, slope=0.0, clamp_lo=clamp[0], clamp_hi=clamp[1])
     flops = 2.0 * n * h * w * pw.cin_real * pw.cout * 9
-    if use_exit:
+    if z_add is not None:
+        _dev_check(z_add, "z_add")
+        if not use_exit or c not in (64, 96) or tuple(z_add.shape) != (n, h, w, 32):
+            raise ValueError(f"z_add {tuple(z_add.shape)}: the additive map is [N, H, W, 32] for the taps-as-rows exit kernel with 64 or 96 "
+                             f"input channels (x {tuple(x.shape)}, rows form {use_exit})")
+        _timed_call(lib.virnet_conv_exit_add, (C.byref(d), nat.ptr(z_add)), "conv_exit(z_add)", ("exit", pw.cout), flops)
+    elif use_exit:
         _timed_call(lib.virnet_conv_exit, (C.byref(d),), "conv_exit", ("exit", pw.cout), flops)
     else:
         _timed_call(lib.virnet_conv_f16, (C.byref(d),), "conv_f16(nchw)", ("f16x3", pw.cout), flops)
     return out
+
+
+def compose_exit_weight(w2: Tensor, b2: Optional[Tensor], w_exit: Tensor) -> PackedWeight:
+    w2, w_exit = w2.detach(), w_exit.detach()
+    b2 = None if b2 is None else b2.detach()
+    for t, nm in ((w2, "w2"), (b2, "b2"), (w_exit, "w_exit")):
+        if t is not None:
+            _dev_check(t, nm)
+    ce, cm = w_exit.shape[:2]
+    if tuple(w_exit.shape[2:]) != (3, 3) or tuple(w2.shape[2:]) != (3, 3) or w2.shape[0] != cm or ce * 9 > 32:
+        raise ValueError(f"compose_exit_weight: exit {tuple(w_exit.shape)} over conv {tuple(w2.shape)}: 3x3 kernels, matching channels and "
+                         f"at most 3 exit channels")
+    ci = w2.shape[1]
+    wc = torch.empty((32, ci, 3, 3), dtype=torch.float32, device=w2.device)
+    bc = torch.empty(32, dtype=torch.float32, device=w2.device)
+    nat.check(nat.load().virnet_compose_exit_weight(nat.ptr(w2), nat.ptr(b2), nat.ptr(w_exit), ce, cm, ci, nat.ptr(wc), nat.ptr(bc),
+                                                    nat.stream_handle()), "compose_exit_weight")
+    return pack_weight(wc, bc)
 
 
 def pack_thin_weight(weight: Tensor, bias: Optional[Tensor]) -> PackedWeight:
```

After: 1585 (median of 6 runs). 1.01x the previous value.
